# bobg/bs

Hardware: AMD Instinct MI355X
Metric: GiB/s device-resident split+ref-hash; chunk/ref bit-parity vs Go ref (higher is better)
Workload: dtype u8

## Files before the change

bs_amd/bsgpu.py:

```python
from __future__ import annotations

import contextlib
import ctypes
import os
import re

import numpy as np

_HERE = os.path.dirname(os.path.abspath(__file__))
LIB_PATH = os.environ.get("BSG_LIB_PATH") or os.path.join(_HERE, "libbsgpu.so")
HEADER_PATH = os.path.join(os.path.dirname(_HERE), "include", "bsgpu.h")

BSG_OK = 0
READ_SLACK = 256
ERRORS = {-22: "EINVAL", -12: "ENOMEM", -5: "EDEVICE", -71: "ESTATE", -19: "ENODEV",
          -2: "ENOTFOUND", -74: "ECORRUPT", -1001: "EIO"}


class BsgError(RuntimeError):
    def __init__(self, code: int, what: str = "", info: dict | None = None):
        self.code = code
        self.info = info
        super().__init__(f"{what}: bsgpu error {code} ({ERRORS.get(code, '?')})")

# ... 175 lines not shown
        return np.ascontiguousarray(ranges)
    out = np.zeros(len(ranges), dtype=READ_RANGE_DTYPE)
    for q, (root, offset, n) in enumerate(ranges):
        out[q]["root"] = np.frombuffer(bytes(root), dtype=np.uint8)
        out[q]["offset"], out[q]["len"] = offset, n
    return out

_lib = None


def exported_symbols_from_header(path: str = HEADER_PATH) -> list[str]:
    text = open(path).read()
    text = re.sub(r"/\*.*?\*/", "", text, flags=re.S)
    return sorted(set(re.findall(r"\b(bsg_[a-z0-9_]+)\s*\(", text)))


def lib() -> ctypes.CDLL:
    global _lib
    if _lib is not None:
        return _lib
    if not os.path.exists(LIB_PATH):
        raise RuntimeError(f"{LIB_PATH} not built: run `python -m bs_amd.build` "
                           "(the HIP path is the only path; there is no CPU fallback)")
    L = ctypes.CDLL(LIB_PATH)
    vp, u8p, u32p, u64p = (ctypes.c_void_p, ctypes.POINTER(ctypes.c_uint8),
                           ctypes.POINTER(ctypes.c_uint32), ctypes.POINTER(ctypes.c_uint64))
    sig = {
        "bsg_errstr": (ctypes.c_char_p, [ctypes.c_int]),
        "bsg_params_default": (Params, []),
        "bsg_default_table": (None, [u32p]),
        "bsg_device_count": (ctypes.c_int, []),
        "bsg_init": (ctypes.c_int, [ctypes.c_int]),
        "bsg_open": (vp, [ctypes.c_int, ctypes.POINTER(Params), u32p, ctypes.POINTER(ctypes.c_int)]),
        "bsg_write": (ctypes.c_int, [vp, vp, ctypes.c_size_t]),
        "bsg_close": (ctypes.c_int, [vp]),
        "bsg_close_begin": (ctypes.c_int, [vp]),
        "bsg_close_step": (ctypes.c_int, [vp, ctypes.POINTER(ctypes.c_size_t)]),
        "bsg_pending": (ctypes.c_size_t, [vp]),
        "bsg_drain": (ctypes.c_size_t, [vp, vp, ctypes.c_size_t]),
        "bsg_set_tile": (ctypes.c_int, [vp, ctypes.c_size_t]),
        "bsg_set_carry_cap": (ctypes.c_int, [vp, ctypes.c_size_t]),
        "bsg_write_window": (ctypes.c_int, [vp, ctypes.POINTER(ctypes.c_void_p),
                                            ctypes.POINTER(ctypes.c_size_t)]),
        "bsg_write_commit": (ctypes.c_int, [vp, ctypes.c_size_t]),
        "bsg_host_register": (ctypes.c_int, [vp, ctypes.c_size_t]),
        "bsg_host_unregister": (ctypes.c_int, [vp]),
        "bsg_write_pinned": (ctypes.c_int, [vp, vp, ctypes.c_size_t]),
        "bsg_free": (None, [vp]),
        "bsg_reset": (ctypes.c_int, [vp]),
        "bsg_engine_create": (vp, [ctypes.c_int, u32p, ctypes.POINTER(ctypes.c_int)]),
        "bsg_engine_destroy": (None, [vp]),
        "bsg_engine_run": (ctypes.c_int, [vp, vp, u64p, u64p, ctypes.c_uint32,
                                          ctypes.POINTER(Params)]),
        "bsg_engine_hash": (ctypes.c_int, [vp, vp, u64p, u64p, ctypes.c_uint32]),
        "bsg_engine_finish": (ctypes.c_int, [vp, u64p]),
        "bsg_engine_chunks_device": (vp, [vp]),
        "bsg_engine_copy_chunks": (ctypes.c_int, [vp, vp, ctypes.c_uint64]),
        "bsg_engine_copy_counts": (ctypes.c_int, [vp, u64p, ctypes.c_uint32]),
        "bsg_engine_stream": (vp, [vp]),
        "bsg_engine_trees": (ctypes.c_int, [vp, u64p, u64p]),
        "bsg_engine_copy_roots": (ctypes.c_int, [vp, vp, u64p, ctypes.c_uint32]),
        "bsg_engine_copy_tree_nodes": (ctypes.c_int, [vp, vp, ctypes.c_uint64, vp,
                                                      ctypes.c_uint64]),
        "bsg_engine_tree_nodes_device": (vp, [vp]),
        "bsg_engine_tree_arena_device": (vp, [vp]),
        "bsg_engine_roots_device": (vp, [vp]),
        "bsg_engine_trees_ms_debug": (ctypes.c_int, [vp, ctypes.POINTER(ctypes.c_float)]),
        "bsg_refset_new": (vp, [ctypes.c_int, ctypes.POINTER(ctypes.c_int)]),
        "bsg_refset_free": (None, [vp]),
        "bsg_refset_count": (ctypes.c_uint64, [vp]),
        "bsg_refset_add": (ctypes.c_int, [vp, vp, ctypes.c_uint64, vp]),
        "bsg_engine_dedup": (ctypes.c_int, [vp, vp, u64p, u64p]),
        "bsg_engine_copy_dedup": (ctypes.c_int, [vp, vp, ctypes.c_uint64, vp, vp,
                                                 ctypes.c_uint64]),
        "bsg_engine_dedup_first_device": (vp, [vp]),
        "bsg_engine_dedup_uniq_device": (vp, [vp]),
        "bsg_engine_dedup_pack_off_device": (vp, [vp]),
        "bsg_engine_pack_unique": (ctypes.c_int, [vp, vp, ctypes.c_uint64]),
        "bsg_engine_dedup_ms_debug": (ctypes.c_int, [vp, ctypes.POINTER(ctypes.c_float)]),
        "bsg_engine_restore": (ctypes.c_int, [vp, vp, ctypes.c_uint64, vp, ctypes.c_uint64, vp,
                                              ctypes.c_uint64, vp, ctypes.c_uint64, u64p, u64p,
                                              ctypes.c_uint32, ctypes.c_int,
                                              ctypes.POINTER(RestoreInfo)]),
        "bsg_engine_restore_ms_debug": (ctypes.c_int, [vp, ctypes.POINTER(ctypes.c_float)]),
        "bsg_engine_walk": (ctypes.c_int, [vp, vp, ctypes.c_uint64, vp, ctypes.c_uint64, vp,
                                           ctypes.c_uint32, ctypes.c_int, vp,
                                           ctypes.POINTER(WalkInfo)]),
        "bsg_engine_copy_walk": (ctypes.c_int, [vp, vp, ctypes.c_uint64, vp, vp,
                                                ctypes.c_uint32]),
        "bsg_engine_walk_records_device": (vp, [vp]),
        "bsg_engine_restore_walk": (ctypes.c_int, [vp, vp, ctypes.c_uint64, vp, ctypes.c_uint64,
                                                   vp, ctypes.c_uint64, u64p, ctypes.c_uint32,
                                                   ctypes.c_int, ctypes.POINTER(RestoreInfo)]),
        "bsg_engine_walk_ms_debug": (ctypes.c_int, [vp, ctypes.POINTER(ctypes.c_float)]),
        "bsg_engine_gc_mark": (ctypes.c_int, [vp, vp, ctypes.c_uint64, vp, ctypes.c_uint64, vp,
                                              ctypes.c_uint64, ctypes.c_int, vp,
                                              ctypes.POINTER(GcInfo)]),
        "bsg_engine_copy_gc": (ctypes.c_int, [vp, vp, ctypes.c_uint64, vp, ctypes.c_uint64,
                                              ctypes.c_int]),
        "bsg_engine_gc_live_device": (vp, [vp]),
        "bsg_engine_gc_compact": (ctypes.c_int, [vp, vp, ctypes.c_uint64, vp, ctypes.c_uint64,
                                                 ctypes.c_int, u64p]),
        "bsg_engine_gc_ms_debug": (ctypes.c_int, [vp, ctypes.POINTER(ctypes.c_float)]),
        "bsg_pool_new": (vp, [ctypes.c_int, ctypes.c_uint64, ctypes.c_uint64,
                              ctypes.POINTER(ctypes.c_int)]),
        "bsg_pool_free": (None, [vp]),
        "bsg_pool_stat": (ctypes.c_int, [vp, ctypes.POINTER(PoolStats)]),
        "bsg_pool_bytes_device": (vp, [vp]),
        "bsg_pool_table_device": (vp, [vp]),
        "bsg_pool_copy_table": (ctypes.c_int, [vp, vp, ctypes.c_uint64, ctypes.c_uint64]),
        "bsg_engine_pool_put": (ctypes.c_int, [vp, vp, ctypes.c_int,
                                               ctypes.POINTER(POOL_PUT_INFO)]),
        "bsg_pool_copy_where": (ctypes.c_int, [vp, vp, ctypes.c_uint64]),
        "bsg_pool_where_device": (vp, [vp]),
        "bsg_pool_put_ms_debug": (ctypes.c_int, [vp, ctypes.POINTER(ctypes.c_float)]),
        "bsg_pool_collect": (ctypes.c_int, [vp, vp, vp, vp, ctypes.c_uint64, ctypes.c_int, vp,
                                            ctypes.POINTER(PoolCollectInfo)]),
        "bsg_pool_copy_remap": (ctypes.c_int, [vp, vp, ctypes.c_uint64]),
        "bsg_pool_remap_device": (vp, [vp]),
        "bsg_pool_reset": (ctypes.c_int, [vp]),
        "bsg_pool_walk": (ctypes.c_int, [vp, vp, vp, ctypes.c_uint32, ctypes.c_int, vp,
                                         ctypes.POINTER(WalkInfo)]),
        "bsg_pool_restore_walk": (ctypes.c_int, [vp, vp, vp, ctypes.c_uint64, u64p,
                                                 ctypes.c_uint32, ctypes.c_int,
                                                 ctypes.POINTER(RestoreInfo)]),
        "bsg_engine_read": (ctypes.c_int, [vp, vp, ctypes.c_uint64, vp, ctypes.c_uint64, vp,
                                           ctypes.c_uint32, vp, ctypes.c_uint64, vp, ctypes.c_int,
                                           vp, vp, ctypes.POINTER(ReadInfo)]),
        "bsg_pool_read": (ctypes.c_int, [vp, vp, vp, ctypes.c_uint32, vp, ctypes.c_uint64, vp,
                                         ctypes.c_int, vp, vp, ctypes.POINTER(ReadInfo)]),
        "bsg_pool_kill_debug": (ctypes.c_int, [vp]),
        "bsg_engine_read_ms_debug": (ctypes.c_int, [vp, ctypes.POINTER(ctypes.c_float)]),
        "bsg_pool_collect_ms_debug": (ctypes.c_int, [vp, ctypes.POINTER(ctypes.c_float)]),
        "bsg_pool_merge": (ctypes.c_int, [vp, vp, vp, vp, ctypes.c_uint64, ctypes.c_int, vp,
                                          ctypes.POINTER(PoolMergeInfo)]),
        "bsg_pool_sync": (ctypes.c_int, [vp, vp, vp, ctypes.c_int, ctypes.POINTER(PoolMergeInfo)]),
        "bsg_pool_merge_ms_debug": (ctypes.c_int, [vp, ctypes.c_int,
                                                   ctypes.POINTER(ctypes.c_float)]),
        "bsg_pool_put_blobs": (ctypes.c_int, [vp, vp, vp, u64p, u64p, ctypes.c_uint64,
                                              ctypes.c_int, vp, ctypes.POINTER(POOL_PUT_INFO)]),
        "bsg_pool_get": (ctypes.c_int, [vp, vp, vp, ctypes.c_uint64, vp, ctypes.c_uint64,
                                        ctypes.c_int, vp, vp, ctypes.POINTER(PoolGetInfo)]),
        "bsg_pool_blobs_ms_debug": (ctypes.c_int, [vp, ctypes.POINTER(ctypes.c_float)]),
        "bsg_engine_pack_mode_debug": (ctypes.c_int, [vp, ctypes.c_int]),
        "bsg_engine_d2d_ms_debug": (ctypes.c_int, [vp, vp, vp, ctypes.c_uint64,
                                                   ctypes.POINTER(ctypes.c_float)]),
        "bsg_engine_candidates": (ctypes.c_uint64, [vp]),
        "bsg_engine_profile": (ctypes.c_int, [vp, ctypes.c_int]),
        "bsg_engine_diag": (ctypes.c_int, [vp, u64p]),
        "bsg_engine_timeline": (ctypes.c_int, [vp, u64p]),
        "bsg_engine_tiers_debug": (ctypes.c_int, [vp, u64p]),
        "bsg_engine_early_min_debug": (ctypes.c_int, [vp, ctypes.c_uint64]),
        "bsg_engine_host_tail": (ctypes.c_int, [vp, u64p]),
        "bsg_engine_host_tail_debug": (ctypes.c_int, [vp, ctypes.c_uint64, ctypes.c_uint32,
                                                      ctypes.c_int, ctypes.c_uint64]),
        "bsg_host_sha256_debug": (ctypes.c_int, [vp, ctypes.c_uint64, ctypes.c_int, vp]),
        "bsg_engine_early_picks_debug": (ctypes.c_int, [vp, u64p]),
        "bsg_engine_rescan_debug": (ctypes.c_uint64, [vp]),
        "bsg_engine_regions_debug": (ctypes.c_int, [vp, vp, ctypes.c_uint64]),
        "bsg_engine_stage_ms": (ctypes.c_int, [vp, ctypes.POINTER(ctypes.c_float)]),
        "bsg_split_hash_batch": (ctypes.c_int, [ctypes.c_int, vp, u64p, u64p, ctypes.c_uint32,
                                                ctypes.POINTER(Params), u32p, vp,
                                                ctypes.c_uint64, u64p, u64p]),
        "bsg_sha256_batch": (ctypes.c_int, [ctypes.c_int, vp, u64p, u64p, ctypes.c_uint32, vp]),
        "bsg_hasher_new": (vp, [ctypes.c_int]),
        "bsg_hasher_sum": (ctypes.c_int, [vp, vp, u64p, u64p, ctypes.c_uint32, vp]),
        "bsg_hasher_sum_ptrs": (ctypes.c_int, [vp, ctypes.POINTER(ctypes.c_void_p), u64p,
                                               ctypes.c_uint32, vp]),
        "bsg_hasher_free": (None, [vp]),
        "bsg_hasher_pinned_bytes": (ctypes.c_size_t, [vp]),
        "bsg_fill_splitmix": (ctypes.c_int, [ctypes.c_int, vp, ctypes.c_uint64, ctypes.c_uint64,
                                             vp]),
        "bsg_device_malloc": (vp, [ctypes.c_int, ctypes.c_size_t]),
        "bsg_device_free": (ctypes.c_int, [ctypes.c_int, vp]),
        "bsg_memcpy": (ctypes.c_int, [ctypes.c_int, vp, vp, ctypes.c_size_t, ctypes.c_int]),
        "bsg_device_synchronize": (ctypes.c_int, [ctypes.c_int]),
        "bsg_memstore_new": (vp, [ctypes.c_int]),
        "bsg_filestore_new": (vp, [ctypes.c_char_p, ctypes.c_int]),
        "bsg_store_free": (None, [vp]),
        "bsg_store_count": (ctypes.c_size_t, [vp]),
        "bsg_filestore_set_write_behind": (ctypes.c_int, [vp, ctypes.c_uint64]),
        "bsg_store_held_bytes": (ctypes.c_size_t, [vp]),
        "bsg_store_get": (ctypes.c_int, [vp, vp, vp, ctypes.c_size_t,
                                         ctypes.POINTER(ctypes.c_size_t)]),
        "bsg_store_put": (ctypes.c_int, [vp, vp, ctypes.c_size_t, vp,
                                         ctypes.POINTER(ctypes.c_int)]),
        "bsg_store_list": (ctypes.c_size_t, [vp, vp, ctypes.c_size_t]),
        "bsg_store_put_ref": (ctypes.c_int, [vp, vp, vp, ctypes.c_size_t,
                                             ctypes.POINTER(ctypes.c_int)]),
        "bsg_store_list_from": (ctypes.c_size_t, [vp, vp, vp, ctypes.c_size_t]),
        "bsg_store_delete": (ctypes.c_int, [vp, vp]),
        "bsg_split_protect": (ctypes.c_int, [vp, vp, vp, vp, ctypes.c_size_t,
                                             ctypes.POINTER(ctypes.c_size_t)]),
        "bsg_writer_new": (vp, [ctypes.c_int, vp, ctypes.POINTER(Params), ctypes.c_size_t,
                                ctypes.POINTER(ctypes.c_int)]),
        "bsg_writer_write": (ctypes.c_int, [vp, vp, ctypes.c_size_t]),
        "bsg_writer_close": (ctypes.c_int, [vp]),
        "bsg_writer_root": (ctypes.c_int, [vp, vp]),
        "bsg_writer_timings": (ctypes.c_int, [vp, ctypes.POINTER(ctypes.c_double)]),
        "bsg_stream_stats_get": (ctypes.c_int, [vp, ctypes.POINTER(StreamStats)]),
        "bsg_writer_free": (None, [vp]),
        "bsg_reader_new": (vp, [vp, vp, ctypes.POINTER(ctypes.c_int)]),
        "bsg_reader_open": (vp, [vp, vp, ctypes.c_int, ctypes.c_int, ctypes.POINTER(ctypes.c_int)]),
        "bsg_reader_read": (ctypes.c_int64, [vp, vp, ctypes.c_size_t]),
        "bsg_reader_seek": (ctypes.c_int64, [vp, ctypes.c_int64, ctypes.c_int]),
        "bsg_reader_size": (ctypes.c_uint64, [vp]),
        "bsg_reader_stats": (ctypes.c_int, [vp, u64p]),
        "bsg_debug_set": (ctypes.c_int, [ctypes.c_int, ctypes.c_int64]),
        "bsg_debug_get": (ctypes.c_int64, [ctypes.c_int]),
        "bsg_set_stream_base": (ctypes.c_int, [vp, ctypes.c_uint64]),
        "bsg_writer_set_stream_base": (ctypes.c_int, [vp, ctypes.c_uint64]),
        "bsg_reader_free": (None, [vp]),
    }
    partial = os.environ.get("BSG_LIB_PARTIAL") == "1"
    for name, (res, args) in sig.items():
        if partial and not hasattr(L, name):
            continue
        f = getattr(L, name)
        f.restype = res
        f.argtypes = args
    _lib = L
    return L


def _check(rc: int, what: str) -> None:
    if rc != BSG_OK:
        raise BsgError(rc, what)


def _as_u8(data) -> np.ndarray:
    if isinstance(data, np.ndarray):
        return np.ascontiguousarray(data.reshape(-1).view(np.uint8))
    return np.frombuffer(data, dtype=np.uint8)


def _u64(a) -> np.ndarray:
    return np.ascontiguousarray(np.asarray(a, dtype=np.uint64))


def _p(a: np.ndarray, ct):
    return a.ctypes.data_as(ctypes.POINTER(ct))


(KNOB_SEQ_WAIT, KNOB_LONG_MODE, KNOB_VERIFY_WINDOW, KNOB_EARLY, KNOB_POLL, KNOB_COPY_NT,
 KNOB_LIGHT_BYTES, KNOB_HOST_TAIL) = range(1, 9)


def debug_get(knob: int) -> int:
    return int(lib().bsg_debug_get(knob))


def debug_set(knob: int, value: int) -> None:
    _check(lib().bsg_debug_set(knob, value), "bsg_debug_set")


@contextlib.contextmanager
def debug_knob(knob: int, value: int):
    old = debug_get(knob)
    debug_set(knob, value)
    try:
        yield
    finally:
        debug_set(knob, old)


def device_count() -> int:
    return lib().bsg_device_count()


def init(device: int = 0) -> None:
    _check(lib().bsg_init(device), "bsg_init")


def default_table() -> np.ndarray:
    t = np.zeros(256, dtype=np.uint32)
    lib().bsg_default_table(_p(t, ctypes.c_uint32))
    return t


def params(bits: int = 16, min_size: int = 1024, fanout: int = 8) -> Params:
    return Params(bits, min_size, fanout, 0)


def _table_arg(table):
    if table is None:
        return None, None
    t = np.ascontiguousarray(np.asarray(table, dtype=np.uint32))
    assert t.shape == (256,)
    return t, _p(t, ctypes.c_uint32)


def split_hash_batch(streams: list[bytes] | list[np.ndarray], bits: int = 16,
                     min_size: int = 1024, table=None, device: int = 0):
    arrs = [np.frombuffer(bytes(s), dtype=np.uint8) if not isinstance(s, np.ndarray)
            else np.ascontiguousarray(s, dtype=np.uint8) for s in streams]
    lens = _u64([len(a) for a in arrs])
    off = _u64(np.concatenate([[0], np.cumsum(lens)[:-1]]) if len(arrs) else [])
    base = np.concatenate(arrs) if arrs else np.zeros(1, np.uint8)
    if base.size == 0:
        base = np.zeros(1, np.uint8)
    cap = int(sum(int(l) // (min_size or 64) + 2 for l in lens)) + 1
    out = np.zeros(cap, dtype=CHUNK_DTYPE)
    counts = np.zeros(max(len(arrs), 1), dtype=np.uint64)
    n = ctypes.c_uint64(0)
    p = params(bits, min_size)
    _t, tp = _table_arg(table)
# ... 349 lines not shown
                   cap: int | None = None):
        pp = pool.ptr if isinstance(pool, DeviceBuffer) else pool
        op = out.ptr if isinstance(out, DeviceBuffer) else out
        pool_bytes = pool.nbytes + READ_SLACK if pool_bytes is None else pool_bytes
        cap = out.nbytes if cap is None else cap
        n = ctypes.c_uint64(0)
        rc = lib().bsg_engine_gc_compact(self.h, pp, pool_bytes, op, cap,
                                         GC_ALIGN16 if align16 else 0, ctypes.byref(n))
        return rc, n.value

    def gc_ms(self) -> dict:
        out = (ctypes.c_float * 4)()
        _check(lib().bsg_engine_gc_ms_debug(self.h, out), "bsg_engine_gc_ms_debug")
        return {"index": float(out[0]), "levels": float(out[1]), "offsets": float(out[2]),
                "compact": float(out[3])}

    def pool_put(self, pool: "Pool", chunks: bool = True, nodes: bool = True) -> dict:
        flags = (POOL_CHUNKS if chunks else 0) | (POOL_NODES if nodes else 0)
        info = POOL_PUT_INFO()
        rc = lib().bsg_engine_pool_put(self.h, pool.h, flags, ctypes.byref(info))
        if rc != BSG_OK:
            raise BsgError(rc, "bsg_engine_pool_put", info.as_dict())
        pool._items = int(info.items)
        return info.as_dict()

    def pool_collect(self, src: "Pool", dst: "Pool", roots, flags: int = 0):
        roots = np.ascontiguousarray(np.frombuffer(roots, dtype=np.uint8)
                                     if isinstance(roots, (bytes, bytearray)) else roots,
                                     dtype=np.uint8).reshape(-1)
        assert len(roots) % 32 == 0
        nr = len(roots) // 32
        status = np.zeros(max(nr, 1), dtype=np.int32)
        info = PoolCollectInfo()
        nsrc = src.stat()["nblobs"] if src is not None and src.h else 0
        rc = lib().bsg_pool_collect(self.h, src.h if src is not None else None,
                                    dst.h if dst is not None else None, roots.ctypes.data, nr,
                                    flags, status.ctypes.data, ctypes.byref(info))
        self._gc_nblobs, self._gc_nlive = nsrc, int(info.gc.nlive)
        if rc == BSG_OK:
            dst._nremap = nsrc
        return rc, info.as_dict(), status[:nr]

    def pool_merge(self, src: "Pool", dst: "Pool", roots=None, all: bool = False,
                   verify: bool = False, missing_leaves: bool = False):
        if roots is None:
            rp, nr = None, 0
        else:
            roots = np.ascontiguousarray(np.frombuffer(roots, dtype=np.uint8)
                                         if isinstance(roots, (bytes, bytearray)) else roots,
                                         dtype=np.uint8).reshape(-1)
            assert len(roots) % 32 == 0
            rp, nr = roots.ctypes.data, len(roots) // 32
        flags = ((MERGE_ALL if all else 0) | (MERGE_VERIFY if verify else 0)
                 | (GC_MISSING_LEAVES if missing_leaves else 0))
        status = np.zeros(max(nr, 1), dtype=np.int32)
        info = PoolMergeInfo()
        nsrc = src.stat()["nblobs"] if src is not None and src.h else 0
        rc = lib().bsg_pool_merge(self.h, src.h if src is not None else None,
                                  dst.h if dst is not None else None, rp, nr, flags,
                                  status.ctypes.data, ctypes.byref(info))
        if not all:
            self._gc_nblobs, self._gc_nlive = nsrc, int(info.gc.nlive)
        if rc == BSG_OK:
            dst._nremap = nsrc
        return rc, info.as_dict(), status[:nr]

    def pool_sync(self, a: "Pool", b: "Pool", verify: bool = False):
        info = (PoolMergeInfo * 2)()
        na = a.stat()["nblobs"] if a is not None and a.h else 0
        nb = b.stat()["nblobs"] if b is not None and b.h else 0
        rc = lib().bsg_pool_sync(self.h, a.h if a is not None else None,
                                 b.h if b is not None else None, MERGE_VERIFY if verify else 0,
                                 info)
        if rc == BSG_OK:
            b._nremap, a._nremap = na, nb
        return rc, [info[0].as_dict(), info[1].as_dict()], np.zeros(0, dtype=np.int32)

    def pool_merge_ms(self, direction: int = 0) -> dict:
        out = (ctypes.c_float * 5)()
        _check(lib().bsg_pool_merge_ms_debug(self.h, direction, out), "bsg_pool_merge_ms_debug")
        return dict(zip(("probe", "plan", "verify", "append", "gather"), map(float, out)))

    def pool_walk(self, pool: "Pool", roots, flags: int = 0):
        roots = np.ascontiguousarray(np.frombuffer(roots, dtype=np.uint8)
                                     if isinstance(roots, (bytes, bytearray)) else roots,
                                     dtype=np.uint8).reshape(-1)
        assert len(roots) % 32 == 0
        ns = len(roots) // 32
        status = np.zeros(max(ns, 1), dtype=np.int32)
        info = WalkInfo()
        rc = lib().bsg_pool_walk(self.h, pool.h if pool is not None else None, roots.ctypes.data,
                                 ns, flags, status.ctypes.data, ctypes.byref(info))
        self._walk_ns, self._walk_nrecs = ns, int(info.nrecs)
        return rc, info.as_dict(), status[:ns]

    def pool_restore_walk(self, pool: "Pool", out, out_off, verify: bool = False,
                          out_cap: int | None = None):
        op = out.ptr if isinstance(out, DeviceBuffer) else out
        out_cap = out.nbytes if out_cap is None else out_cap
        oo = _u64(out_off)
        info = RestoreInfo()
        rc = lib().bsg_pool_restore_walk(self.h, pool.h if pool is not None else None, op, out_cap,
                                         _p(oo, ctypes.c_uint64), len(oo),
                                         RESTORE_VERIFY if verify else 0, ctypes.byref(info))
        return rc, info.as_dict()

    def read(self, pool, blobs, ranges, out, out_off, flags: int = 0,
             pool_bytes: int | None = None, out_cap: int | None = None):
        pp = pool.ptr if isinstance(pool, DeviceBuffer) else pool
        op = out.ptr if isinstance(out, DeviceBuffer) else out
        pool_bytes = pool.nbytes + READ_SLACK if pool_bytes is None else pool_bytes
        out_cap = out.nbytes if out_cap is None else out_cap
        blobs = np.ascontiguousarray(blobs, dtype=POOL_BLOB_DTYPE)
        rg, oo = read_ranges(ranges), _u64(out_off)
        assert len(rg) == len(oo)
        status = np.zeros(max(len(rg), 1), dtype=np.int32)
        got = np.zeros(max(len(rg), 1), dtype=np.uint64)
        info = ReadInfo()
        rc = lib().bsg_engine_read(self.h, pp, pool_bytes, blobs.ctypes.data, len(blobs),
                                   rg.ctypes.data, len(rg), op, out_cap, oo.ctypes.data, flags,
                                   status.ctypes.data, got.ctypes.data, ctypes.byref(info))
        return rc, status[:len(rg)], got[:len(rg)], info.as_dict()

    def read_ms(self) -> dict:
        out = (ctypes.c_float * 6)()
        _check(lib().bsg_engine_read_ms_debug(self.h, out), "bsg_engine_read_ms_debug")
        return dict(zip(("index", "levels", "placement", "resolve", "verify", "scatter"),
                        (float(x) for x in out)))

    def dedup_ms(self) -> dict:
        out = (ctypes.c_float * 2)()
        _check(lib().bsg_engine_dedup_ms_debug(self.h, out), "bsg_engine_dedup_ms_debug")
        return {"dedup": float(out[0]), "pack": float(out[1])}

    @property
    def stream(self) -> int:
        return lib().bsg_engine_stream(self.h) or 0

    def profile(self, enable: int = 1) -> None:
        _check(lib().bsg_engine_profile(self.h, int(enable)), "bsg_engine_profile")

    def stage_ms(self) -> list[float]:
        out = (ctypes.c_float * 3)()
        _check(lib().bsg_engine_stage_ms(self.h, out), "bsg_engine_stage_ms")
        return [float(x) for x in out]

    def diag(self) -> dict:
        d = np.zeros(16, dtype=np.uint64)
        _check(lib().bsg_engine_diag(self.h, _p(d, ctypes.c_uint64)), "bsg_engine_diag")
        out = {"nlong": int(d[0]), "long_thresh": int(d[1]), "max_nblocks": int(d[2]),
               "nshort": int(d[13]), "wave_tickets": int(d[14]), "total_blocks": int(d[15])}
        t = np.zeros(4, dtype=np.uint64)
        _check(lib().bsg_engine_timeline(self.h, _p(t, ctypes.c_uint64)), "bsg_engine_timeline")
        if t[0] and t[1] and t[3]:
            t0 = int(t[0])
            out["timeline_us"] = {"long_start": round((int(t[1]) - t0) * 0.01, 1),
                                  "long_end": round((int(t[2]) - t0) * 0.01, 1),
                                  "lane_end": round((int(t[3]) - t0) * 0.01, 1)}
        if os.environ.get("BSG_DIAG_RAW") == "1":
            out["diag2_raw"] = [int(x) for x in d[8:13]]
        for tag, o in (("long", 3), ("lane", 8)):
            cyc, rt, nb = int(d[o + 1] - d[o]), int(d[o + 3] - d[o + 2]), int(d[o + 4])
            if nb and rt:
                out[tag] = {"blocks": nb, "cycles_per_block": round(cyc / nb, 1),
                            "clock_ghz": round(cyc / (rt * 10.0), 3),
                            "us_per_block": round(rt * 0.01 / nb, 4)}
        t = np.zeros(12, dtype=np.uint64)
        _check(lib().bsg_engine_host_tail(self.h, _p(t, ctypes.c_uint64)), "bsg_engine_host_tail")
        out["host_tail"] = {"chunks": int(t[0]), "bytes": int(t[1]), "cut_blocks": int(t[2]),
                            "gather_us": int(t[3]), "host_done_us": int(t[4]),
                            "impl": "x86-sha" if int(t[5]) == 1 else "portable",
                            "threads": int(t[6]), "host_rate_bytes_s": int(t[7]),
                            "longest_blocks": int(t[8]), "longest_left_blocks": int(t[9]),
                            "host_blocks": int(t[10]), "cpuid_sha": bool(t[11])}
        return out

    def set_host_tail(self, min_bytes: int = 512 << 20, force_cut: int = 0,
                      portable: bool = False, ring_bytes: int = 0) -> None:
        _check(lib().bsg_engine_host_tail_debug(self.h, int(min_bytes), int(force_cut),
                                                int(bool(portable)), int(ring_bytes)),
               "bsg_engine_host_tail_debug")

    def tiers(self) -> dict:
        d = np.zeros(6, dtype=np.uint64)
        _check(lib().bsg_engine_tiers_debug(self.h, _p(d, ctypes.c_uint64)),
               "bsg_engine_tiers_debug")
        return {"nlong_grp": int(d[0]), "tickets_grp": int(d[1]), "helped": int(d[2]),
                "wave_tickets": int(d[3]), "early": (bool(d[4]), bool(d[5]))}

    def set_early_min(self, nbytes: int) -> None:
        _check(lib().bsg_engine_early_min_debug(self.h, int(nbytes)),
               "bsg_engine_early_min_debug")

    def early_picks(self) -> list:
        d = np.zeros(4, dtype=np.uint64)
        _check(lib().bsg_engine_early_picks_debug(self.h, _p(d, ctypes.c_uint64)),
               "bsg_engine_early_picks_debug")
        out = []
        for k in range(2):
            top, idx = int(d[k]), int(d[2 + k])
            if top:
                out.append((top >> 32, top & 0xFFFFFFFF, idx - 1 if idx else None))
            elif idx:
                raise BsgError(-5, f"bsg_engine_early_picks_debug: idx[{k}] without top[{k}]")
        if not d[0] and d[1]:
            raise BsgError(-5, "bsg_engine_early_picks_debug: top[1] without top[0]")
        return out

    def regions(self) -> dict:
        kmax = 256
        d = np.zeros(8 + kmax + kmax + 1, dtype=np.uint64)
        _check(lib().bsg_engine_regions_debug(self.h, d.ctypes.data, d.nbytes),
               "bsg_engine_regions_debug")
        R = int(d[0])
        if not 1 <= R <= kmax:
            raise BsgError(-5, f"bsg_engine_regions_debug: nregions {R}")
        return {"nregions": R, "off": [int(x) for x in d[8 + kmax: 8 + kmax + R + 1]]}

    @property
    def candidates(self) -> int:
        return lib().bsg_engine_candidates(self.h)

    @property
    def rescan_strips(self) -> int:
        return int(lib().bsg_engine_rescan_debug(self.h))

    def close(self) -> None:
        if self.h:
            lib().bsg_engine_destroy(self.h)
            self.h = None

    def __del__(self):
        try:
            self.close()
        except Exception:
            pass


IN_SET = 1 << 63


class RefSet:

    def __init__(self, device: int = 0):
        err = ctypes.c_int(0)
        self.h = lib().bsg_refset_new(device, ctypes.byref(err))
        if not self.h:
            raise BsgError(err.value, "bsg_refset_new")

    def add(self, refs) -> np.ndarray:
        if not isinstance(refs, np.ndarray):
            refs = np.frombuffer(b"".join(bytes(r) for r in refs), dtype=np.uint8)
        a = np.ascontiguousarray(refs, dtype=np.uint8).reshape(-1, 32)
        added = np.zeros(max(len(a), 1), dtype=np.uint8)
        _check(lib().bsg_refset_add(self.h, a.ctypes.data, len(a), added.ctypes.data),
               "bsg_refset_add")
        return added[: len(a)]

    def count(self) -> int:
        return int(lib().bsg_refset_count(self.h))

    def free(self) -> None:
        if self.h:
            lib().bsg_refset_free(self.h)
            self.h = None

    def __del__(self):
        try:
            self.free()
        except Exception:
            pass


class Pool:

    def __init__(self, cap_bytes: int, cap_blobs: int, device: int = 0):
        err = ctypes.c_int(0)
        self.device, self._items, self._nremap = device, 0, 0
        self.h = lib().bsg_pool_new(device, cap_bytes, cap_blobs, ctypes.byref(err))
        if not self.h:
            raise BsgError(err.value, "bsg_pool_new")

    def stat(self) -> dict:
        st = PoolStats()
        _check(lib().bsg_pool_stat(self.h, ctypes.byref(st)), "bsg_pool_stat")
        return st.as_dict()

    @property
    def ptr(self) -> int:
        return lib().bsg_pool_bytes_device(self.h) or 0

    @property
    def pool_bytes(self) -> int:
        return self.stat()["pool_bytes"]

    def table(self, first: int = 0) -> np.ndarray:
        n = self.stat()["nblobs"] - first
        out = np.zeros(max(n, 1), dtype=POOL_BLOB_DTYPE)
        _check(lib().bsg_pool_copy_table(self.h, out.ctypes.data, first, max(n, 0)),
               "bsg_pool_copy_table")
        return out[:max(n, 0)]

    def where(self) -> np.ndarray:
        out = np.zeros(max(self._items, 1), dtype=np.uint64)
        _check(lib().bsg_pool_copy_where(self.h, out.ctypes.data, self._items),
               "bsg_pool_copy_where")
        return out[:self._items]

    def to_host(self, n: int | None = None) -> np.ndarray:
        n = self.stat()["bytes"] if n is None else n
        out = np.empty(max(n, 1), dtype=np.uint8)
        if n:
            _check(lib().bsg_memcpy(self.device, out.ctypes.data, self.ptr, n, 1), "bsg_memcpy")
        return out[:n]

    def read(self, eng: "Engine", ranges, out, out_off, flags: int = 0,
             out_cap: int | None = None):
        op = out.ptr if isinstance(out, DeviceBuffer) else out
        out_cap = out.nbytes if out_cap is None else out_cap
        rg, oo = read_ranges(ranges), _u64(out_off)
        assert len(rg) == len(oo)
        status = np.zeros(max(len(rg), 1), dtype=np.int32)
        got = np.zeros(max(len(rg), 1), dtype=np.uint64)
        info = ReadInfo()
        rc = lib().bsg_pool_read(eng.h if eng is not None else None, self.h, rg.ctypes.data,
                                 len(rg), op, out_cap, oo.ctypes.data, flags, status.ctypes.data,
                                 got.ctypes.data, ctypes.byref(info))
        return rc, status[:len(rg)], got[:len(rg)], info.as_dict()
# ... 372 lines not shown
```

bs_amd/csrc/bsgpu_host.cpp:

```cpp
#include <hip/hip_runtime.h>
#include <pthread.h>
#include <sched.h>
#include <sys/mman.h>
#include <sys/syscall.h>
#include <unistd.h>

#include <emmintrin.h>

#include <algorithm>
#include <atomic>
#include <chrono>
#include <condition_variable>
#include <cstdio>
#include <cstdlib>
#include <cstring>
#include <deque>
#include <functional>
#include <memory>
#include <mutex>
#include <new>
#include <thread>
#include <vector>

#include "../../include/bsgpu.h"
// ... 868 lines not shown
  HCHECK(hipEventCreate(&a));
  if (hipEventCreate(&b) != hipSuccess) {
    (void)hipGetLastError();
    (void)hipEventDestroy(a);
    return BSG_EDEVICE;
  }
  hipError_t err = hipEventRecord(a, e->stream);
  if (err == hipSuccess)
    err = hipMemcpyDtoDAsync((hipDeviceptr_t)dst, (hipDeviceptr_t)src, n, e->stream);
  if (err == hipSuccess) err = hipEventRecord(b, e->stream);
  if (err == hipSuccess) err = hipStreamSynchronize(e->stream);
  if (err == hipSuccess) err = hipEventElapsedTime(ms, a, b);
  (void)hipEventDestroy(a);
  (void)hipEventDestroy(b);
  if (err != hipSuccess) (void)hipGetLastError();
  return herr(err);
}

bsg_refset* bsg_refset_new(int device, int* err) {
  int dummy;
  if (!err) err = &dummy;
  if (device < 0 || device >= bsg_device_count()) {
    *err = BSG_ENODEV;
    return nullptr;
  }
  bsg_refset* s = new (std::nothrow) bsg_refset();
  if (!s) {
    *err = BSG_ENOMEM;
    return nullptr;
  }
  s->dev = device;
  *err = BSG_EDEVICE;
  if (hipSetDevice(device) == hipSuccess && stream_acquire(device, &s->stream) == hipSuccess) {
    s->num_cus = device_cus(device);
    s->slots = kRefSetSlots0;
    s->key_cap = kRefSetSlots0;
    *err = BSG_ENOMEM;
    if (s->tab.ensure(8 * s->slots) == hipSuccess && s->keys.ensure(32 * s->key_cap) == hipSuccess) {
      *err = herr(hipMemset(s->tab.p, 0xFF, 8 * s->slots));
      if (*err == BSG_OK) return s;
    }
  }
  (void)hipGetLastError();
  bsg_refset_free(s);
  return nullptr;
}

void bsg_refset_free(bsg_refset* s) {
  if (!s) return;
  hipSetDevice(s->dev);
  if (s->stream) {
    hipStreamSynchronize(s->stream);
    stream_release(s->dev, s->stream);
  }
  delete s;
}

uint64_t bsg_refset_count(const bsg_refset* s) { return s ? s->count.load() : 0; }

int bsg_refset_add(bsg_refset* s, const uint8_t* refs, uint64_t n, uint8_t* added) {
  if (!s || (n && !refs) || n > (1ull << 40)) return BSG_EINVAL;
  std::lock_guard<std::mutex> g(s->mu);
  if (s->dead) return BSG_ESTATE;
  HCHECK(hipSetDevice(s->dev));
  if (!n) return BSG_OK;
  int rc;
  if ((rc = s->work.reserve(n))) return rc;
  MCHECK(s->staged.ensure(32 * n));
  HCHECK(hipMemcpyAsync(s->staged.p, refs, 32 * n, hipMemcpyHostToDevice, s->stream));
  HCHECK(hipMemsetAsync(s->work.hdr.p, 0, sizeof(DedupHdr), s->stream));
  HCHECK(s->work.tab.clear(s->stream));
  DedupArgs a = s->work.args(s->staged.as<uint8_t>(), 32, nullptr, 0, n);
  s->lookup_args(&a);
  HCHECK(dbg("launch_dedup", s->stream, launch_dedup(a, s->stream, s->num_cus)));
  if ((rc = s->work.readback(s->stream))) {
    if (rc == BSG_EDEVICE) s->dead = true;
    return rc;
  }
  const uint64_t m = s->work.last.nunique;
  if (m > n) {
    s->dead = true;
    return BSG_EDEVICE;
  }
  std::vector<uint64_t> first;
  if (added) {
    try {
      first.resize(n);
    } catch (const std::bad_alloc&) {
      return BSG_ENOMEM;
    }
    HCHECK(hipMemcpy(first.data(), s->work.first.p, 8 * n, hipMemcpyDeviceToHost));
  }
  if ((rc = s->add_new(a, m, &s->work, s->stream))) return rc;
  if (added)
    for (uint64_t i = 0; i < n; ++i) added[i] = first[i] == i ? 1 : 0;
  return BSG_OK;
}

int bsg_engine_profile(bsg_engine* e, int enable) {
  if (!e || enable < 0 || enable > 2) return BSG_EINVAL;
  int rc = e->setdev();
  if (rc) return rc;
  if (enable) HCHECK(e->marks.create(4));
  e->profile = enable;
  return BSG_OK;
}

int bsg_engine_stage_ms(const bsg_engine* e, float out[3]) {
  if (!e || !out || !e->profile) return BSG_EINVAL;
  for (int i = 0; i < 3; ++i) out[i] = e->stage_ms[i];
  return BSG_OK;
}

uint64_t bsg_engine_candidates(const bsg_engine* e) { return e ? e->last.ncand : 0; }

int bsg_engine_diag(const bsg_engine* e, uint64_t out[16]) {
  if (!e || !out) return BSG_EINVAL;
  out[0] = e->last.nlong;
  out[1] = e->last.long_thresh;
  out[2] = e->last.max_nblocks;
  for (int i = 0; i < 5; ++i) out[3 + i] = e->last.diag[i];
  for (int i = 0; i < 5; ++i) out[8 + i] = e->last.diag2[i];
  out[13] = e->last.nshort;
  out[14] = e->last.ntickets;
  out[15] = e->last.total_blocks;
  return BSG_OK;
}

int bsg_engine_host_tail(const bsg_engine* e, uint64_t out[12]) {
  if (!e || !out) return BSG_EINVAL;
  const bsg_engine::TailStat& t = e->tail_stat;
  out[0] = t.chunks;
  out[1] = t.bytes;
  out[2] = t.cut;
  out[3] = (uint64_t)(t.gather_ms > 0 ? t.gather_ms * 1000.f : 0.f);
  out[4] = (uint64_t)std::max<int64_t>(0, t.host_done_us);
  out[5] = (uint64_t)t.impl;
  out[6] = (uint64_t)t.threads;
  out[7] = (uint64_t)t.host_rate;
  out[8] = t.longest_all;
  out[9] = t.longest_left;
  out[10] = t.blocks;
  out[11] = sha256_have_x86() ? 1 : 0;
  return BSG_OK;
}

extern "C" int bsg_engine_host_tail_debug(bsg_engine* e, uint64_t min_bytes, uint32_t force_cut,
                                          int portable, uint64_t ring_bytes) {
  if (!e || e->enqueued || (ring_bytes && ring_bytes < 4096)) return BSG_EINVAL;
  e->tail_min = min_bytes;
  e->tail_force_cut = force_cut;
  e->tail_portable = portable != 0;
  e->tail_ring_force = ring_bytes;
  return BSG_OK;
}

extern "C" int bsg_engine_regions_debug(bsg_engine* e, void* out, uint64_t nbytes) {
  if (!e || !out || !e->regions.p) return BSG_EINVAL;
  if (e->setdev()) return BSG_EDEVICE;
  const uint64_t n = std::min<uint64_t>(nbytes, sizeof(Regions));
  if (hipStreamSynchronize(e->stream) != hipSuccess) return BSG_EDEVICE;
  return hipMemcpy(out, e->regions.p, n, hipMemcpyDeviceToHost) == hipSuccess ? BSG_OK : BSG_EDEVICE;
}

static int read_early(bsg_engine* e, Early* ea) {
  if (e->hash_mode || !e->ctr.p || e->ctr.cap < sizeof(Counters) + sizeof(Early)) return BSG_OK;
  if (e->setdev() || hipStreamSynchronize(e->stream) != hipSuccess ||
      hipMemcpy(ea, e->dearly(), sizeof(Early), hipMemcpyDeviceToHost) != hipSuccess)
    return BSG_EDEVICE;
  return BSG_OK;
}

extern "C" int bsg_engine_tiers_debug(bsg_engine* e, uint64_t out[6]) {
  if (!e || !out || e->enqueued) return BSG_EINVAL;
  out[0] = e->last.nlong_grp;
  out[1] = e->last.tickets_grp;
  out[2] = e->last.helped;
  out[3] = e->last.ntickets;
  Early ea{};
  const int rc = read_early(e, &ea);
  for (int k = 0; k < kEarly; ++k) out[4 + k] = (ea.top[k] && ea.idx[k]) ? 1 : 0;
  return rc;
}

extern "C" int bsg_engine_early_min_debug(bsg_engine* e, uint64_t bytes) {
  if (!e || e->enqueued) return BSG_EINVAL;
  e->early_min = bytes;
  return BSG_OK;
}

extern "C" int bsg_engine_early_picks_debug(bsg_engine* e, uint64_t out[4]) {
  if (!e || !out || e->enqueued) return BSG_EINVAL;
  Early ea{};
  const int rc = read_early(e, &ea);
  for (int k = 0; k < kEarly; ++k) {
    out[k] = ea.top[k];
    out[kEarly + k] = ea.idx[k];
  }
  return rc;
}

extern "C" uint64_t bsg_engine_rescan_debug(const bsg_engine* e) {
  return e && !e->enqueued ? e->last.rescan : ~0ull;
}

extern "C" int bsg_engine_trees_ms_debug(const bsg_engine* e, float out[4]) {
  if (!e || !out) return BSG_EINVAL;
  if (!e->profile || !e->tree.valid) return BSG_ESTATE;
  for (int i = 0; i < 4; ++i) out[i] = e->tree.ms[i];
  return BSG_OK;
}

int bsg_engine_timeline(const bsg_engine* e, uint64_t out[4]) {
  if (!e || !out) return BSG_EINVAL;
  out[0] = e->last.sha_start_rt;
  out[1] = e->last.diag[2];
  out[2] = e->last.diag[3];
  out[3] = e->last.lane_end_rt;
  return BSG_OK;
}

bsg_ctx* bsg_open(int device, const bsg_params* params, const uint32_t* table, int* err) {
  int dummy;
  if (!err) err = &dummy;
  Params p;
  bsg_params norm;
  int rc = normalize(params, &p, &norm);
  if (rc) {
    *err = rc;
    return nullptr;
  }
  if (device < 0 || device >= bsg_device_count()) {
    *err = BSG_ENODEV;
    return nullptr;
  }
  bsg_ctx* c = new (std::nothrow) bsg_ctx();
  if (!c) {
    *err = BSG_ENOMEM;
    return nullptr;
  }
  c->params = norm;
  c->p = p;
  if (hipSetDevice(device) != hipSuccess || (rc = c->init(device, table)) != BSG_OK) {
    delete c;
    *err = rc ? rc : BSG_EDEVICE;
    return nullptr;
  }
  *err = BSG_OK;
  return c;
}

int bsg_set_tile(bsg_ctx* c, size_t tile) {
  if (!c || tile < 4096 || c->fill || c->pos != c->stream0 || c->started) return BSG_EINVAL;
  c->tile = tile;
  return BSG_OK;
}

int bsg_set_carry_cap(bsg_ctx* c, size_t bytes) {
  if (!c || c->fill || c->pos != c->stream0 || c->started || bytes > 0xffffffffull)
    return BSG_EINVAL;
  c->carry_cap = bytes;
  return BSG_OK;
}

int bsg_set_stream_base(bsg_ctx* c, uint64_t base) {
  if (!c || c->fill || c->pos != c->stream0 || c->started || c->closed) return BSG_EINVAL;
  c->stream0 = c->pos = base;
  return BSG_OK;
}

static int ctx_write(bsg_ctx* c, const uint8_t* p, size_t n,
                     int (bsg_ctx::*write)(const uint8_t*, size_t)) {
  if (!c) return BSG_EINVAL;
  if (c->closed) return BSG_ESTATE;
  if (c->sticky) return c->sticky;
  if (n && !p) return BSG_EINVAL;
  if (hipSetDevice(c->dev) != hipSuccess) return BSG_EDEVICE;
  c->started = true;
  int rc = (c->*write)(p, n);
  if (rc) c->sticky = rc;
  return rc;
}

int bsg_write(bsg_ctx* c, const uint8_t* p, size_t n) { return ctx_write(c, p, n, &bsg_ctx::write); }

int bsg_host_register(void* p, size_t n) {
  if (!p || !n) return BSG_EINVAL;
  HCHECK(hipHostRegister(p, n, hipHostRegisterDefault));
  return BSG_OK;
}

int bsg_host_unregister(void* p) {
  if (!p) return BSG_EINVAL;
  HCHECK(hipHostUnregister(p));
  return BSG_OK;
}

int bsg_write_pinned(bsg_ctx* c, const uint8_t* p, size_t n) {
  return ctx_write(c, p, n, &bsg_ctx::write_pinned);
}

int bsg_write_window(bsg_ctx* c, uint8_t** p, size_t* cap) {
  if (!c || !p || !cap) return BSG_EINVAL;
  if (c->closed) return BSG_ESTATE;
  if (c->sticky) return c->sticky;
  if (hipSetDevice(c->dev) != hipSuccess) return BSG_EDEVICE;
// ... 316 lines not shown
```

bs_amd/csrc/bsgpu_internal.h:

```cpp
#pragma once
#include <stddef.h>
#include <stdint.h>

namespace bsg {

constexpr int kScanWG = 512;
#ifndef BSG_STRIP
#define BSG_STRIP 2048
#endif
constexpr int kStrip = BSG_STRIP;
constexpr int kSlotCap = 4;
constexpr int kTabRows = 256;
constexpr int kTabRep = 64;

constexpr int kCandPosShift = 8;
constexpr uint64_t kCandPosMask = (1ull << 40) - 1;
constexpr uint64_t kCandForce = 1ull << 7;

__host__ __device__ inline uint64_t cand_pack(uint32_t stream, uint64_t pos, bool force,
                                              uint32_t tz) {
  return ((uint64_t)stream << 48) | ((pos & kCandPosMask) << kCandPosShift) |
         (force ? kCandForce : 0ull) | (uint64_t)(tz & 63u);
}
__host__ __device__ inline uint32_t cand_stream(uint64_t c) { return (uint32_t)(c >> 48); }
__host__ __device__ inline uint64_t cand_pos(uint64_t c) {
  return (c >> kCandPosShift) & kCandPosMask;
}
__host__ __device__ inline bool cand_force(uint64_t c) { return (c & kCandForce) != 0; }
__host__ __device__ inline uint32_t cand_tz(uint64_t c) { return (uint32_t)(c & 63u); }

__host__ __device__ inline uint32_t slot_pack(uint32_t local, bool force, uint32_t tz) {
  return (local << 8) | (force ? 0x80u : 0u) | (tz & 63u);
}

struct StreamDesc {
  uint64_t data_off;
  uint64_t len;
  uint64_t strip0;
  uint64_t seg_base;
  uint64_t open_start;
  uint64_t consumed;
  uint32_t finalize;
  uint32_t prefix_len;
  uint32_t mid[8];
  uint32_t carry_cap;
  uint32_t flags;
  uint8_t hist[64];
};
constexpr uint32_t kDescOpenInDevice = 1;
static_assert(sizeof(StreamDesc) == 160, "StreamDesc layout");

struct CarryOut {
  uint32_t mid[8];
  uint64_t consumed;
  uint64_t open_start;
  uint32_t prefix_len;
  uint32_t valid;
};

struct ChunkRec {
  uint64_t offset;
  uint64_t len;
  uint32_t level;
  uint32_t stream;
  uint8_t ref[32];
};
static_assert(sizeof(ChunkRec) == 56, "ChunkRec layout");

struct Params {
  uint32_t split_bits;
  uint32_t min_size;
  uint32_t mask;
  uint32_t pad_;
};

struct Counters {
  uint64_t ncand;
  uint64_t nchunks;
  uint64_t help_wg;
  uint64_t overflow;
  uint64_t error;
  uint64_t max_nblocks;
  uint64_t long_thresh;
  uint64_t nlong;
  uint64_t long_head;
  uint64_t nshort;
  uint64_t bucket_width;
  uint64_t diag[5];
  uint64_t diag2[5];
  uint64_t rescan;
  uint64_t total_blocks;
  uint64_t long_buckets;
  uint64_t ntickets;
  uint64_t sha_arrivals;
  uint64_t sha_start_rt;
  uint64_t lane_end_rt;
  uint64_t nlong_grp;
  uint64_t tickets_grp;
  uint64_t nrefine;
  uint64_t helped;
  uint64_t scan_ticket;
  uint64_t pad[7];
};
static_assert(sizeof(Counters) == 320, "Counters layout");

struct LaneJob {
  uint64_t dptr;
  uint64_t start;
  uint64_t len;
  uint32_t stream;
  uint32_t meta;
};
static_assert(sizeof(LaneJob) == 32, "LaneJob layout");
constexpr uint32_t kLaneJobSlow = 0x80000000u;

constexpr uint32_t kMaxRegions = 256;
constexpr uint32_t kRegionSegs = 256;
constexpr uint32_t kMinRegionJobs = 4096;
constexpr uint64_t kRegionBytes = 1ull << 30;
struct Regions {
  uint64_t nregions;
  uint64_t rr;
  uint64_t pad_[6];
  uint64_t head[kMaxRegions];
  uint64_t off[kMaxRegions + 1];
  uint64_t pad2_[7];
  uint32_t cnt[kRegionSegs * kMaxRegions];
};

constexpr int kEarly = 2;
struct Early {
  uint64_t top[kEarly];
  uint64_t idx[kEarly];
  uint64_t diag[5];
  uint64_t pad_;
  ChunkRec rec[kEarly];
};
static_assert(sizeof(Early) % 16 == 0, "Early layout");

constexpr uint32_t kTailBuckets = 256;
constexpr uint32_t kTailMaxItems = 4096;
constexpr uint32_t kTailMinBlocks = 256;
constexpr uint32_t kTailSlotAlign = 256;
struct TailItem {
  uint64_t job;
  uint64_t start;
  uint64_t len;
  uint64_t off;
  uint32_t stream;
  uint32_t level;
};
static_assert(sizeof(TailItem) == 40, "TailItem layout");
struct TailHdr {
  uint64_t count;
  uint64_t cutb;
  uint64_t bytes;
  uint64_t blocks;
  uint64_t mx_all;
  uint64_t mx_left;
  uint64_t ring_head;
  uint64_t taken;
  uint32_t cnt[kTailBuckets];
  uint32_t maxb[kTailBuckets];
  uint64_t rbytes[kTailBuckets];
  uint64_t nblk[kTailBuckets];
  uint32_t base[kTailBuckets];
  uint32_t fill[kTailBuckets];
};
static_assert(sizeof(TailHdr) % 16 == 0, "TailHdr layout");
constexpr uint32_t kTailMetaWords = 8;
__host__ __device__ inline uint64_t tail_slot(uint64_t len) {
  return (len + 16 + kTailSlotAlign - 1) & ~(uint64_t)(kTailSlotAlign - 1);
}

constexpr uint32_t kLongMinBlocks = 1024;
#ifndef BSG_SOLO
#define BSG_SOLO 16
#endif
constexpr uint32_t kSolo = BSG_SOLO;
constexpr uint32_t kGroup = 8;
constexpr uint32_t kPairGroup = 32;
constexpr int kLongRow = 68;
constexpr int kRingWords = 65 * kLongRow;
constexpr int kLptBuckets = 4096;
constexpr uint64_t kReadSlack = 256;

constexpr uint32_t kTreeMaxHeights = 40;
struct TreeNode {
  uint64_t blob_off;
  uint32_t blob_len;
  uint32_t stream;
  uint32_t height;
  uint32_t reserved;
  uint8_t ref[32];
};
static_assert(sizeof(TreeNode) == 56, "TreeNode layout");
struct TreeHdr {
  uint64_t nnodes;
  uint64_t arena_bytes;
  uint64_t max_r;
  uint64_t error;
  uint64_t hoff[kTreeMaxHeights + 1];
};
struct TreeNodeMeta {
  uint64_t child0;
  uint64_t nchild;
  uint64_t offset, size;
  uint64_t out_idx;
  uint64_t blob_off;
  uint32_t blob_len;
  uint32_t stream;
};

constexpr uint64_t kDedupEmpty = ~0ull;
constexpr uint64_t kDedupInSet = 1ull << 63;
constexpr uint64_t kRefSetSlots0 = 1024;
constexpr uint64_t kRefSetLoadPct = 50;
constexpr uint32_t kPackTile = 32768;
struct DedupHdr {
  uint64_t error;
  uint64_t nunique;
  uint64_t unique_bytes;
  uint64_t pad_;
};

constexpr uint32_t kRestoreTile = 32768;
struct PoolBlob {
  uint64_t off;
  uint64_t len;
  uint8_t ref[32];
};
static_assert(sizeof(PoolBlob) == 48, "PoolBlob layout");
struct RestoreHdr {
  DedupHdr dd;
  uint64_t invalid;
  uint64_t missing;
  uint64_t mismatch;
  uint64_t bad_blob;
};
static_assert(sizeof(RestoreHdr) == 64, "RestoreHdr layout");

constexpr uint32_t kWalkMaxDepth = 64;
constexpr uint32_t kWalkRuns = 12;
constexpr uint64_t kWalkDead = ~0ull;
constexpr uint32_t kWalkCorrupt = 1;
constexpr uint32_t kWalkNotFound = 2;
struct WalkItem {
  uint64_t blob;
  uint64_t exp_off;
  uint64_t exp_size;
  uint64_t parent;
  uint32_t stream;
  uint32_t flags;
};
constexpr uint32_t kWalkNoCover = 1;
static_assert(sizeof(WalkItem) == 40, "WalkItem layout");
struct WalkNode {
  uint64_t nchild;
  uint64_t offset, size;
  uint64_t nrec;
  uint64_t rbase;
  uint32_t kind;
  uint32_t nruns;
  uint64_t run_pos[kWalkRuns];
  uint64_t run_idx[kWalkRuns];
  uint32_t run_len[kWalkRuns];
};
struct WalkHdr {
  DedupHdr dd;
  uint64_t nnodes;
  uint64_t depth;
  uint64_t lvl_all[kWalkMaxDepth + 1];
  uint64_t lvl_nodes[kWalkMaxDepth + 1];
};
static_assert(sizeof(WalkHdr) % 16 == 0, "WalkHdr layout");

struct ReadHdr {
  WalkHdr w;
  RestoreHdr r;
  uint64_t verified;
  uint64_t pad_;
};
static_assert(sizeof(ReadHdr) % 16 == 0 && offsetof(ReadHdr, r) % 16 == 0, "ReadHdr layout");

constexpr uint32_t kGcClaimed = 1;
constexpr uint32_t kGcFailed = 2;
constexpr uint32_t kGcTile = 32768;
struct GcHdr {
  WalkHdr w;
  uint64_t bad_form;
  uint64_t bad_miss;
  uint64_t verdict;
  uint64_t leaf_miss;
  uint64_t missing_leaves;
  uint64_t end, end16;
  uint64_t size0;
  uint32_t status0;
  uint32_t pad_;
  uint64_t pad2_;
  uint8_t zero[16];
};
static_assert(sizeof(GcHdr) % 16 == 0 && offsetof(GcHdr, zero) % 16 == 0, "GcHdr layout");

constexpr uint32_t kPoolTile = 32768;
struct PoolHdr {
  DedupHdr dd;
  uint64_t total16;
  uint64_t last_len;
  uint64_t known;
  uint64_t repeats;
  uint8_t zero[16];
};
static_assert(sizeof(PoolHdr) % 16 == 0 && offsetof(PoolHdr, zero) % 16 == 0, "PoolHdr layout");

struct MergeHdr {
  GcHdr g;
  RestoreHdr r;
  uint64_t selected;
  uint64_t known;
  uint64_t added_bytes;
  uint64_t end;
  uint64_t verified;
  uint64_t pad_;
// ... 19 lines not shown
```

bs_amd/csrc/bsgpu_kernels.hip:

```cpp
#include <hip/hip_runtime.h>

#include <algorithm>

#include "bsgpu_internal.h"
#include "bsgpu_launch.h"
#include "sha256_device.h"
#include "scan_block_loop.inc"

#ifndef BSG_TLEN_PCT
#define BSG_TLEN_PCT 55
#endif
#ifndef BSG_PAIR_PCT
#define BSG_PAIR_PCT 34
#endif
#ifndef BSG_TLEN_PCT_LIGHT
#define BSG_TLEN_PCT_LIGHT 48
#endif
#ifndef BSG_PAIR_PCT_LIGHT
#define BSG_PAIR_PCT_LIGHT 30
#endif

namespace bsg {

typedef uint32_t u32x4 __attribute__((ext_vector_type(4), aligned(4)));
// ... 1260 lines not shown

__global__ __launch_bounds__(kRegionSegs) void k_rscan(ShaArgs a) {
  __shared__ uint32_t wsum[kRegionSegs / 64];
  if (a.ctr->overflow || a.ctr->error || a.ctr->nchunks > a.chunk_cap) return;
  const uint32_t r = blockIdx.x, t = threadIdx.x;
  if (r >= a.reg->nregions) return;
  uint32_t* c = a.reg->cnt + t * kMaxRegions + r;
  const uint32_t v = *c;
  uint32_t x = v;
  for (int o = 1; o < 64; o <<= 1) {
    const uint32_t y = __shfl_up(x, o);
    if ((t & 63) >= (uint32_t)o) x += y;
  }
  if ((t & 63) == 63) wsum[t >> 6] = x;
  __syncthreads();
  uint32_t base = 0, tot = 0;
  for (uint32_t w = 0; w < kRegionSegs / 64; ++w) {
    if (w < (t >> 6)) base += wsum[w];
    tot += wsum[w];
  }
  *c = base + x - v;
  if (t == 0) a.reg->head[r] = tot;
}

__global__ __launch_bounds__(kMaxRegions) void k_rtotal(ShaArgs a) {
  __shared__ uint64_t wsum[kMaxRegions / 64];
  if (a.ctr->overflow || a.ctr->error || a.ctr->nchunks > a.chunk_cap) return;
  const uint32_t t = threadIdx.x;
  const uint32_t R = (uint32_t)a.reg->nregions;
  const uint64_t v = t < R ? a.reg->head[t] : 0;
  uint64_t x = v;
  for (int o = 1; o < 64; o <<= 1) {
    const uint64_t y = __shfl_up(x, o);
    if ((t & 63) >= (uint32_t)o) x += y;
  }
  if ((t & 63) == 63) wsum[t >> 6] = x;
  __syncthreads();
  uint64_t base = 0;
  for (uint32_t w = 0; w < (t >> 6); ++w) base += wsum[w];
  __syncthreads();
  a.reg->off[t] = t < R ? base + x - v : a.ctr->nshort;
  if (t == 0) {
    a.reg->off[kMaxRegions] = a.ctr->nshort;
    a.reg->rr = 0;
  }
  a.reg->head[t] = 0;
}

__global__ __launch_bounds__(256) void k_rscatter(ShaArgs a) {
  __shared__ uint64_t base[kMaxRegions];
  __shared__ uint32_t tc[kMaxRegions];
  if (a.ctr->overflow || a.ctr->error || a.ctr->nchunks > a.chunk_cap) return;
  const uint64_t n = a.ctr->nshort, L = seg_len(n);
  const uint32_t t = threadIdx.x;
  base[t] = a.reg->off[t] + a.reg->cnt[blockIdx.x * kMaxRegions + t];
  tc[t] = 0;
  __syncthreads();
  const uint64_t lo = blockIdx.x * L, hi = min(n, lo + L);
  for (uint64_t tile = lo; tile < hi; tile += 256) {
    const uint64_t i = tile + t;
    uint32_t r = 0, rank = 0;
    uint64_t j = 0;
    if (i < hi) {
      r = a.oreg[i];
      j = a.order[i];
      rank = atomicAdd(&tc[r], 1u);
    }
    __syncthreads();
    if (i < hi) a.rorder[base[r] + rank] = j;
    __syncthreads();
    base[t] += tc[t];
    tc[t] = 0;
    __syncthreads();
  }
}

__global__ __launch_bounds__(1024) void k_bucket_scan(ShaArgs a) {
  __shared__ uint32_t wsum[16];
  __shared__ uint32_t nok;
  const uint32_t t = threadIdx.x;
  if (t == 0) nok = 0;
  const uint64_t mx = a.ctr->max_nblocks, w = a.ctr->bucket_width;
  const bool light = a.ctr->total_blocks * 10ull < mx * 64ull * a.waves;
  uint64_t tlen = (mx * (light ? BSG_TLEN_PCT_LIGHT : BSG_TLEN_PCT)) / 100;
  const uint64_t share = (a.ctr->total_blocks * 9) / (10ull * 64ull * a.waves);
  tlen = max(max(tlen, share), (uint64_t)kLongMinBlocks);
  uint64_t cap = kSolo + (uint64_t)kGroup * (a.waves / 2 > kSolo ? a.waves / 2 - kSolo : 0);
  if (a.long_mode == 2) { tlen = 0; cap = ~0ull; }
  uint32_t e[4], pe[4];
#pragma unroll
  for (int i = 0; i < 4; ++i) e[i] = a.bucket_elig[4 * t + i];
  block_scan4(e, pe, wsum);
  uint32_t ok = 0;
#pragma unroll
  for (int i = 0; i < 4; ++i) {
    const uint64_t b = 4 * t + i;
    const uint64_t top = mx > b * w ? mx - b * w : 0;
    ok += (a.long_mode != 1 && top >= tlen && (uint64_t)pe[i] + e[i] <= cap) ? 1u : 0u;
  }
  __syncthreads();
  atomicAdd(&nok, ok);
  __syncthreads();
  const uint32_t nlb8 = nok;
  uint32_t lv[4], lo[4], sv[4], so[4];
#pragma unroll
  for (int i = 0; i < 4; ++i) lv[i] = (4 * t + i < nlb8) ? e[i] : 0u;
  const uint32_t n8 = block_scan4(lv, lo, wsum);
  const uint64_t t8 = n8 <= kSolo ? n8 : kSolo + (n8 - kSolo + kGroup - 1) / kGroup;
  uint32_t nlb = nlb8;
  const uint64_t pair_pct = light ? BSG_PAIR_PCT_LIGHT : BSG_PAIR_PCT;
  if (pair_pct > 0 && a.long_mode == 0) {
    const uint64_t tlen2 = max((mx * pair_pct) / 100, (uint64_t)kLongMinBlocks);
    const uint64_t tb = a.waves / 2 > t8 ? a.waves / 2 - t8 : 0;
    const uint64_t cap2 = tb * kPairGroup;
    uint32_t ok2 = 0;
#pragma unroll
    for (int i = 0; i < 4; ++i) {
      const uint64_t b = 4 * t + i;
      const uint64_t top = mx > b * w ? mx - b * w : 0;
      ok2 += (b >= nlb8 && top >= tlen2 && (uint64_t)pe[i] + e[i] - n8 <= cap2) ? 1u : 0u;
    }
    __syncthreads();
    if (t == 0) nok = 0;
    __syncthreads();
    atomicAdd(&nok, ok2);
    __syncthreads();
    nlb = nlb8 + nok;
#pragma unroll
    for (int i = 0; i < 4; ++i) lv[i] = (4 * t + i < nlb) ? e[i] : 0u;
  }
  const uint32_t nlong = block_scan4(lv, lo, wsum);
#pragma unroll
  for (int i = 0; i < 4; ++i) sv[i] = a.bucket_cnt[4 * t + i] - lv[i];
  const uint32_t nshort = block_scan4(sv, so, wsum);
#pragma unroll
  for (int i = 0; i < 4; ++i) {
    a.bucket_loff[4 * t + i] = lo[i];
    a.bucket_off[4 * t + i] = so[i];
  }
  if (t == 0) {
    a.ctr->long_buckets = nlb;
    a.ctr->nlong = nlong;
    a.ctr->nshort = nshort;
    const uint64_t rmax = min((uint64_t)kMaxRegions, max((uint64_t)a.waves / 16, (uint64_t)1));
    const uint64_t rspan = (a.span + kRegionBytes - 1) / kRegionBytes;
    a.reg->nregions = min(min(rmax, rspan), max((uint64_t)nshort / kMinRegionJobs, (uint64_t)1));
    if (a.span <= kRegionBytes) {
      a.reg->off[0] = 0;
      a.reg->off[1] = nshort;
      a.reg->head[0] = 0;
    }
    a.ctr->long_thresh = mx > (uint64_t)nlb * w ? mx - (uint64_t)nlb * w : 0;
    a.ctr->nlong_grp = n8;
    a.ctr->tickets_grp = t8;
    const uint64_t helped = (light && a.long_mode == 0)
                                ? min(min((uint64_t)n8, (uint64_t)kSolo), (uint64_t)a.waves / 2)
                                : 0;
    a.ctr->helped = helped;
    a.ctr->long_head = helped;
    a.ctr->ntickets = t8 + (nlong - n8 + kPairGroup - 1) / kPairGroup;
  }
}

__device__ __forceinline__ bool early_key(const ShaArgs& a, int k, uint32_t* s, uint64_t* start,
                                          uint64_t* end) {
  const uint64_t top = a.early->top[k];
  if (!top) return false;
  const uint64_t c = a.cand[(uint32_t)top], cn = a.cand[(uint32_t)top + 1];
  *s = cand_stream(c);
  const uint64_t sb = a.streams[*s].seg_base;
  *start = sb + cand_pos(c) + 1;
  *end = sb + cand_pos(cn) + 1;
  return true;
}

__global__ __launch_bounds__(256) void k_lens(ShaArgs a) {
  if (a.ctr->overflow || a.ctr->error) return;
  const uint64_t M = a.ctr->nchunks;
  if (M > a.chunk_cap) return;
  const uint64_t njobs = M + a.nstreams;
  const uint64_t stride = (uint64_t)gridDim.x * blockDim.x;
  uint32_t st[8];
  ShaJob jb;
  uint64_t mx = 0, tot = 0;
  uint32_t es[kEarly] = {~0u, ~0u};
  uint64_t e0[kEarly] = {0, 0}, e1[kEarly] = {0, 0};
  if (a.early)
    for (int k = 0; k < kEarly; ++k)
      if (!early_key(a, k, &es[k], &e0[k], &e1[k])) es[k] = ~0u;
  for (uint64_t j = (uint64_t)blockIdx.x * blockDim.x + threadIdx.x; j < njobs; j += stride) {
    uint32_t info = kNoJob;
    if (sha_setup(a, j, M, jb, st)) {
      tot += jb.nblocks;
      if (jb.prefix == 0) mx = max(mx, (uint64_t)jb.nblocks);
      bool early = false;
      if (j < M && jb.fin && jb.prefix == 0 && jb.consumed == 0)
        for (int k = 0; k < kEarly; ++k)
          if (jb.stream == es[k] && jb.start == e0[k] && jb.end == e1[k]) {
            a.early->idx[k] = j + 1;
            early = true;
          }
      if (early) {
        a.jinfo[j] = kNoJob;
        continue;
      }
      info = min(jb.nblocks, ~kJobElig) | (jb.prefix == 0 ? kJobElig : 0u);
      LaneJob d;
      d.dptr = reinterpret_cast<uint64_t>(jb.dbase);
      d.start = jb.start;
      d.len = jb.L;
      d.stream = jb.stream;
      d.meta = jb.level | ((jb.fin && jb.prefix == 0 && jb.consumed == 0) ? 0u : kLaneJobSlow);
      a.jdesc[j] = d;
    }
    a.jinfo[j] = info;
  }
  __shared__ uint64_t wmx[4], wtot[4];
  for (int o = 32; o > 0; o >>= 1) {
    mx = max(mx, (uint64_t)__shfl_down(mx, o));
    tot += (uint64_t)__shfl_down(tot, o);
  }
  if ((threadIdx.x & 63) == 0) {
    wmx[threadIdx.x >> 6] = mx;
    wtot[threadIdx.x >> 6] = tot;
  }
  __syncthreads();
  if (threadIdx.x == 0) {
    for (int w = 1; w < 4; ++w) {
      mx = max(mx, wmx[w]);
      tot += wtot[w];
    }
    if (mx) atomicMax(reinterpret_cast<unsigned long long*>(&a.ctr->max_nblocks), (unsigned long long)mx);
    if (tot) atomicAdd(reinterpret_cast<unsigned long long*>(&a.ctr->total_blocks), (unsigned long long)tot);
  }
}

__global__ void k_thresh(Counters* ctr, int mode) {
  (void)mode;
  const uint64_t w = (ctr->max_nblocks + kLptBuckets) / kLptBuckets;
  ctr->bucket_width = w ? w : 1;
}

__device__ __forceinline__ void ring_sync() {
  __builtin_amdgcn_fence(__ATOMIC_SEQ_CST, "wavefront");
  __builtin_amdgcn_wave_barrier();
}

__device__ __forceinline__ uint32_t wave_max(uint32_t v) {
  for (int o = 32; o > 0; o >>= 1) v = max(v, (uint32_t)__shfl_xor((int)v, o));
  return v;
}

__device__ void sha_wave_job(const ShaArgs& a, uint64_t M, uint64_t t, uint64_t nlong,
                             uint32_t* ring) {
  const uint32_t lane = threadIdx.x & 63u;
  const uint64_t n8 = a.ctr->nlong_grp, t8 = a.ctr->tickets_grp;
  const bool pairs = t >= t8;
  const bool solo = !pairs && t < kSolo;
  const uint64_t j0 = solo ? t : pairs ? n8 + (t - t8) * kPairGroup : kSolo + (t - kSolo) * kGroup;
  const uint64_t jend = pairs ? nlong : n8;
  const uint32_t G = solo ? 1u : pairs ? kPairGroup : kGroup;
  const uint32_t B = 64u / G;
  const uint32_t cA = lane / B;
  const uint32_t cR = cA;
  ShaJob ja;
  uint32_t sta[8];
  const bool va = j0 + cA < jend && sha_setup(a, a.long_list[j0 + cA], M, ja, sta);
  if (!va) {
    ja.dbase = a.data;
    ja.L = 0;
    ja.fin = 0;
    ja.consumed = 0;
  }
  const uint32_t na = va ? ja.nblocks : 0u;
  ShaJob jb;
  uint32_t st[8];
  const bool vb = j0 + cR < jend && sha_setup(a, a.long_list[j0 + cR], M, jb, st);
  const uint32_t nb = vb ? jb.nblocks : 0u;
  uint64_t tm0 = 0, tr0 = 0;
  const bool stamp = t == 0 && !(a.early && a.early->top[0]);
  if (stamp) {
    tm0 = __builtin_amdgcn_s_memtime();
    tr0 = __builtin_amdgcn_s_memrealtime();
  }
  const uint32_t nmax = __builtin_amdgcn_readfirstlane(wave_max(nb));
  const SkewLane bl = skew_lane();
  const OctLane ol = oct_lane();
  const bool a_side = pairs ? bl.a_side : ol.a_side;
  uint32_t hs[4];
  hs[0] = a_side ? st[0] : st[6];
  hs[1] = a_side ? st[1] : st[7];
  hs[2] = a_side ? st[2] : st[4];
  hs[3] = a_side ? st[3] : st[5];
  RawBlock rb;
  raw_load(ja.dbase, 64ull * min(lane % B, max(na, 1u) - 1u), 0, ja.L, rb);
  for (uint32_t base = 0; base < nmax; base += B) {
    const uint32_t blk = min(base + lane % B, max(na, 1u) - 1u);
    uint32_t W[16];
    raw_to_words(rb, W);
    const int32_t valid = rb.valid;
    raw_load(ja.dbase, 64ull * min(base + B + lane % B, max(na, 1u) - 1u), 0, ja.L, rb);
    if (valid < 64) {
      pad_words(valid, W);
      if (ja.fin && blk + 1 == na) {
        const uint64_t bits = (ja.consumed + ja.L) * 8ull;
        W[14] = (uint32_t)(bits >> 32);
        W[15] = (uint32_t)bits;
      }
    }
    u32x4a* row = reinterpret_cast<u32x4a*>(ring + lane * kLongRow);
#pragma unroll
    for (int tt = 0; tt < 64; tt += 4) {
      uint32_t kw[4];
#pragma unroll
      for (int u = 0; u < 4; ++u) {
        const int i = tt + u;
        if (i >= 16) {
          const uint32_t w15 = W[(i - 15) & 15], w2 = W[(i - 2) & 15];
          const uint32_t s0 = xor3(rotr(w15, 7), rotr(w15, 18), w15 >> 3);
          const uint32_t s1 = xor3(rotr(w2, 17), rotr(w2, 19), w2 >> 10);
          W[i & 15] = (W[i & 15] + s0) + (W[(i - 7) & 15] + s1);
        }
        kw[u] = kK256[i] + W[i & 15];
      }
      row[tt / 4] = u32x4a{kw[0], kw[1], kw[2], kw[3]};
    }
    ring_sync();
    const uint32_t steps = min(B, nmax - base);
    const uint32_t* ones = ring + 64 * kLongRow;
    const uint32_t* krow = a_side ? ones : ring + cR * B * kLongRow;
    const uint32_t stride = a_side ? 0u : 4u * kLongRow;
    if (pairs)
      sha256_blocks_skew(hs, krow, stride, steps, (int32_t)nb - (int32_t)base, bl);
    else
      sha256_blocks_oct(hs, krow, stride, steps, (int32_t)nb - (int32_t)base, ol);
    ring_sync();
  }
  const int pe = (int)(lane & ~(B - 1u)), pa = (int)((lane & ~(B - 1u)) | (pairs ? 1u : 4u));
#pragma unroll
  for (int k = 0; k < 4; ++k) st[k] = (uint32_t)__shfl((int)hs[k], pa);
  st[6] = (uint32_t)__shfl((int)hs[0], pe);
  st[7] = (uint32_t)__shfl((int)hs[1], pe);
  st[4] = (uint32_t)__shfl((int)hs[2], pe);
  st[5] = (uint32_t)__shfl((int)hs[3], pe);
  if (vb && (lane & (B - 1u)) == 0) {
    sha_finish(a, jb, st);
    if (stamp) {
      a.ctr->diag[1] = __builtin_amdgcn_s_memtime();
      a.ctr->diag[3] = __builtin_amdgcn_s_memrealtime();
      a.ctr->diag[0] = tm0;
      a.ctr->diag[2] = tr0;
      a.ctr->diag[4] = jb.nblocks;
    }
  }
}

__device__ __forceinline__ uint64_t pop_uniform(uint64_t* head) {
  uint32_t lo = 0, hi = 0;
  if ((threadIdx.x & 63u) == 0) {
    const uint64_t t = atomicAdd(reinterpret_cast<unsigned long long*>(head), 1ull);
    lo = (uint32_t)t;
    hi = (uint32_t)(t >> 32);
  }
  lo = __builtin_amdgcn_readlane(lo, 0);
  hi = __builtin_amdgcn_readlane(hi, 0);
  return ((uint64_t)hi << 32) | lo;
}

constexpr uint32_t kHelpHalfWords = 64 * kLongRow;
constexpr uint32_t kHelpOnes = 4 * kHelpHalfWords;
constexpr uint32_t kHelpFlags = kHelpOnes + kLongRow;
constexpr uint32_t kHelpWords = kHelpFlags + 8;
constexpr uint32_t kHelpSlot = 4 * kRingWords;

__device__ __forceinline__ uint32_t lds_seq_load(uint32_t* p) {
  return __hip_atomic_load(p, __ATOMIC_ACQUIRE, __HIP_MEMORY_SCOPE_WORKGROUP);
}
__device__ __forceinline__ void lds_seq_store(uint32_t* p, uint32_t v) {
  __hip_atomic_store(p, v, __ATOMIC_RELEASE, __HIP_MEMORY_SCOPE_WORKGROUP);
}
__device__ bool lds_seq_wait(const ShaArgs& a, uint32_t* p, uint32_t want) {
  for (uint32_t i = 0; i < a.seq_wait_limit; ++i) {
    if ((uint32_t)__builtin_amdgcn_readfirstlane((int)lds_seq_load(p)) == want) return true;
    __builtin_amdgcn_s_sleep(1);
  }
  if ((threadIdx.x & 63u) == 0)
    atomicOr(reinterpret_cast<unsigned long long*>(&a.ctr->error), 8ull);
  return false;
}

__device__ __forceinline__ bool solo_chain_blocks(const ShaArgs& a, uint32_t nb, uint32_t (&st)[8],
                                                  uint32_t* lds, uint32_t c) {
  const uint32_t lane = threadIdx.x & 63u;
  const OctLane ol = oct_lane();
  uint32_t hs[4];
  hs[0] = ol.a_side ? st[0] : st[6];
  hs[1] = ol.a_side ? st[1] : st[7];
  hs[2] = ol.a_side ? st[2] : st[4];
  hs[3] = ol.a_side ? st[3] : st[5];
  uint32_t* fill_seq = lds + kHelpFlags + 2 * c;
  uint32_t* done_seq = lds + kHelpFlags + 4 + 2 * c;
  const uint32_t* ones = lds + kHelpOnes;
  uint32_t f = 0;
  for (uint32_t base = 0; base < nb; base += 64, ++f) {
    const uint32_t h = f & 1u;
    if (!lds_seq_wait(a, fill_seq + h, f / 2 + 1)) return false;
    const uint32_t* krow = ol.a_side ? ones : lds + (2 * c + h) * kHelpHalfWords;
    const uint32_t stride = ol.a_side ? 0u : 4u * kLongRow;
    sha256_blocks_oct_solo(hs, krow, stride, min(64u, nb - base), ol);
    if (lane == 0) lds_seq_store(done_seq + h, f / 2 + 1);
  }
#pragma unroll
  for (int k = 0; k < 4; ++k) st[k] = (uint32_t)__shfl((int)hs[k], 4);
  st[6] = (uint32_t)__shfl((int)hs[0], 0);
  st[7] = (uint32_t)__shfl((int)hs[1], 0);
  st[4] = (uint32_t)__shfl((int)hs[2], 0);
  st[5] = (uint32_t)__shfl((int)hs[3], 0);
  return true;
}

__device__ void sha_solo_chain(const ShaArgs& a, uint64_t M, uint64_t t, uint32_t* lds,
                               uint32_t c) {
  const uint32_t lane = threadIdx.x & 63u;
  ShaJob jb;
  uint32_t st[8];
  const bool vb = sha_setup(a, a.long_list[t], M, jb, st);
  const uint32_t nb = __builtin_amdgcn_readfirstlane(vb ? jb.nblocks : 0u);
  const bool stamp = t == 0 && !(a.early && a.early->top[0]);
  uint64_t tm0 = 0, tr0 = 0;
  if (stamp) {
    tm0 = __builtin_amdgcn_s_memtime();
    tr0 = __builtin_amdgcn_s_memrealtime();
  }
  if (!solo_chain_blocks(a, nb, st, lds, c)) return;
  if (vb && lane == 0) {
    sha_finish(a, jb, st);
    if (stamp) {
      a.ctr->diag[1] = __builtin_amdgcn_s_memtime();
      a.ctr->diag[3] = __builtin_amdgcn_s_memrealtime();
      a.ctr->diag[0] = tm0;
      a.ctr->diag[2] = tr0;
      a.ctr->diag[4] = jb.nblocks;
    }
  }
}

__device__ __forceinline__ void solo_fill_blocks(const ShaArgs& a, ShaJob ja, bool va,
                                                 uint32_t* lds, uint32_t c) {
  const uint32_t lane = threadIdx.x & 63u;
  if (!va) {
    ja.dbase = a.data;
    ja.L = 0;
    ja.fin = 0;
    ja.consumed = 0;
  }
  const uint32_t na = __builtin_amdgcn_readfirstlane(va ? ja.nblocks : 0u);
  uint32_t* fill_seq = lds + kHelpFlags + 2 * c;
  uint32_t* done_seq = lds + kHelpFlags + 4 + 2 * c;
  RawBlock rb;
  raw_load(ja.dbase, 64ull * min(lane, max(na, 1u) - 1u), 0, ja.L, rb);
  uint32_t f = 0;
  for (uint32_t base = 0; base < na; base += 64, ++f) {
    const uint32_t h = f & 1u;
    if (f >= 2 && !lds_seq_wait(a, done_seq + h, f / 2)) return;
    const uint32_t blk = min(base + lane, max(na, 1u) - 1u);
    uint32_t W[16];
    raw_to_words(rb, W);
    const int32_t valid = rb.valid;
    raw_load(ja.dbase, 64ull * min(base + 64u + lane, max(na, 1u) - 1u), 0, ja.L, rb);
    if (valid < 64) {
      pad_words(valid, W);
      if (ja.fin && blk + 1 == na) {
        const uint64_t bits = (ja.consumed + ja.L) * 8ull;
        W[14] = (uint32_t)(bits >> 32);
        W[15] = (uint32_t)bits;
      }
    }
    u32x4a* row = reinterpret_cast<u32x4a*>(lds + (2 * c + h) * kHelpHalfWords + lane * kLongRow);
#pragma unroll
    for (int tt = 0; tt < 64; tt += 4) {
      uint32_t kw[4];
#pragma unroll
      for (int u = 0; u < 4; ++u) {
        const int i = tt + u;
        if (i >= 16) {
          const uint32_t w15 = W[(i - 15) & 15], w2 = W[(i - 2) & 15];
          const uint32_t s0 = xor3(rotr(w15, 7), rotr(w15, 18), w15 >> 3);
          const uint32_t s1 = xor3(rotr(w2, 17), rotr(w2, 19), w2 >> 10);
          W[i & 15] = (W[i & 15] + s0) + (W[(i - 7) & 15] + s1);
        }
        kw[u] = kK256[i] + W[i & 15];
      }
      row[tt / 4] = u32x4a{kw[0], kw[1], kw[2], kw[3]};
    }
    if (lane == 0) lds_seq_store(fill_seq + h, f / 2 + 1);
  }
}

__device__ void sha_solo_fill(const ShaArgs& a, uint64_t M, uint64_t t, uint32_t* lds,
                              uint32_t c) {
  ShaJob ja;
  uint32_t sta[8];
  const bool va = sha_setup(a, a.long_list[t], M, ja, sta);
  solo_fill_blocks(a, ja, va, lds, c);
}

constexpr uint32_t kShaWaves = 4;
constexpr uint32_t kShaBlock = 64 * kShaWaves;

template <bool HELP>
__global__ __launch_bounds__(kShaBlock, 1) void k_sha(ShaArgs a) {
  extern __shared__ __attribute__((aligned(16))) uint32_t lds[];
  if (a.ctr->overflow || a.ctr->error) return;
  if ((a.ctr->helped != 0) != HELP) return;
  const uint64_t M = a.ctr->nchunks;
  if (M > a.chunk_cap) return;
  const uint64_t nlong = a.ctr->nlong;
  if ((threadIdx.x & 63u) == 0) {
    const uint64_t rt = __builtin_amdgcn_s_memrealtime();
    if (atomicAdd(reinterpret_cast<unsigned long long*>(&a.ctr->sha_arrivals), 1ull) == 0)
      a.ctr->sha_start_rt = rt;
  }
  const uint64_t ntickets = a.ctr->ntickets;
  const uint32_t wv = __builtin_amdgcn_readfirstlane(threadIdx.x >> 6);
  uint32_t* ring = lds + wv * kRingWords;
  uint64_t t = ~0ull;
  bool helper_wg = false;
  if constexpr (HELP) {
    if (threadIdx.x == 0)
      lds[kHelpSlot] = (uint32_t)atomicAdd(reinterpret_cast<unsigned long long*>(&a.ctr->help_wg), 1ull);
    __syncthreads();
    const uint64_t helped = a.ctr->helped, hw = lds[kHelpSlot];
    if (hw * 2 < helped) {
      helper_wg = true;
      for (uint32_t i = threadIdx.x; i < (uint32_t)kLongRow; i += blockDim.x) lds[kHelpOnes + i] = 1u;
      if (threadIdx.x < 8) lds[kHelpFlags + threadIdx.x] = 0u;
      __syncthreads();
      const uint32_t c = wv & 1u;
      const uint64_t ht = hw * 2 + c;
      if (ht < helped) {
        __builtin_amdgcn_s_setprio(3);
        if (wv < 2) sha_solo_chain(a, M, ht, lds, c);
        else sha_solo_fill(a, M, ht, lds, c);
        __builtin_amdgcn_s_setprio(0);
      }
    }
  }
  if (!helper_wg) {
    for (uint32_t i = threadIdx.x & 63u; i < (uint32_t)kLongRow; i += 64) ring[64 * kLongRow + i] = 1u;
    t = pop_uniform(&a.ctr->long_head);
  }
  if (t < ntickets) {
    __builtin_amdgcn_s_setprio(3);
    while (t < ntickets) {
      sha_wave_job(a, M, t, nlong, ring);
      t = pop_uniform(&a.ctr->long_head);
    }
    __builtin_amdgcn_s_setprio(0);
  }
  sha_lane_mode(a, M);
  if ((threadIdx.x & 63u) == 0)
    atomicMax(reinterpret_cast<unsigned long long*>(&a.ctr->lane_end_rt),
              (unsigned long long)__builtin_amdgcn_s_memrealtime());
}

__device__ __forceinline__ uint64_t pick_key(const uint64_t* __restrict__ cand, uint64_t n,
                                             uint64_t i, uint64_t minsz) {
  if (i == 0 || i + 1 >= n) return 0;
  const uint64_t c = cand[i];
  const uint64_t cp = cand[i - 1], cn = cand[i + 1];
  const uint32_t s = cand_stream(c);
  if (cand_stream(cp) != s || cand_stream(cn) != s) return 0;
  const uint64_t E = cand_pos(c) + 1, Ep = cand_pos(cp) + 1, En = cand_pos(cn) + 1;
  if (E - Ep < minsz) return 0;
  if (!cand_force(cn) && En - E < minsz) return 0;
  if (cand_force(c)) return 0;
  const uint64_t nb = (En - E + 8) / 64 + 1;
  if (nb < kLongMinBlocks || nb >= (1ull << 31)) return 0;
  return (nb << 32) | i;
}

__device__ __forceinline__ void top2_wave(uint64_t& b1, uint64_t& b2) {
  uint64_t m1 = b1;
  for (int o = 32; o > 0; o >>= 1) m1 = max(m1, (uint64_t)__shfl_xor((long long)m1, o));
  uint64_t m2 = b1 == m1 ? b2 : b1;
  for (int o = 32; o > 0; o >>= 1) m2 = max(m2, (uint64_t)__shfl_xor((long long)m2, o));
  b1 = m1;
  b2 = m2;
}

constexpr uint32_t kPickWGs = 64;
__global__ __launch_bounds__(1024) void k_pick(const uint64_t* __restrict__ cand, Counters* ctr,
                                               uint32_t min_size, Early* e) {
  __shared__ uint64_t wp[2 * 16];
  if (ctr->overflow || ctr->error) return;
  const uint64_t n = ctr->ncand;
  if (n >= (1ull << 32)) return;
  uint64_t b1 = 0, b2 = 0;
  const uint64_t stride = (uint64_t)gridDim.x * blockDim.x;
  for (uint64_t i = (uint64_t)blockIdx.x * blockDim.x + threadIdx.x; i < n; i += stride) {
    const uint64_t key = pick_key(cand, n, i, min_size);
    b2 = max(b2, min(key, b1));
    b1 = max(b1, key);
  }
  top2_wave(b1, b2);
  const uint32_t w = threadIdx.x >> 6, nw = blockDim.x >> 6;
  if ((threadIdx.x & 63u) == 0) {
    wp[2 * w] = b1;
    wp[2 * w + 1] = b2;
  }
  __syncthreads();
  if (w != 0) return;
  const uint32_t l = threadIdx.x;
  b1 = l < 2 * nw ? wp[l] : 0;
  b2 = 0;
  top2_wave(b1, b2);
  if (l == 0 && b1) {
    unsigned long long* t = reinterpret_cast<unsigned long long*>(e->top);
    const uint64_t old = atomicMax(t, (unsigned long long)b1);
    if (old < b1) {
      if (old) atomicMax(t + 1, (unsigned long long)old);
      if (b2) atomicMax(t + 1, (unsigned long long)b2);
    } else {
      atomicMax(t + 1, (unsigned long long)b1);
    }
  }
}

__global__ __launch_bounds__(256, 1) void k_early(ShaArgs a, uint32_t split_bits) {
  extern __shared__ __attribute__((aligned(16))) uint32_t lds[];
  if (a.ctr->overflow || a.ctr->error) return;
  Early* e = a.early;
  const uint32_t wv = __builtin_amdgcn_readfirstlane(threadIdx.x >> 6);
  const uint32_t lane = threadIdx.x & 63u;
  for (uint32_t i = threadIdx.x; i < (uint32_t)kLongRow; i += blockDim.x) lds[kHelpOnes + i] = 1u;
  if (threadIdx.x < 8) lds[kHelpFlags + threadIdx.x] = 0u;
  __syncthreads();
  const uint32_t c = wv & 1u;
  ShaJob jb;
  uint32_t s;
  if (!early_key(a, (int)c, &s, &jb.start, &jb.end)) return;
  const uint64_t cn = a.cand[(uint32_t)e->top[c] + 1];
  const StreamDesc* sd = a.streams + s;
  jb.id = c;
  jb.stream = s;
  jb.level = cand_tz(cn) >= split_bits ? cand_tz(cn) - split_bits : 0u;
  jb.fin = 1;
  jb.prefix = 0;
  jb.consumed = 0;
  jb.dbase = a.data + sd->data_off + (jb.start - sd->seg_base);
  jb.hist = sd->hist + 64;
  jb.L = jb.end - jb.start;
  jb.nblocks = (uint32_t)((jb.L + 8) / 64 + 1);
  __builtin_amdgcn_s_setprio(3);
  if (wv >= 2) {
    solo_fill_blocks(a, jb, true, lds, c);
    return;
  }
  uint32_t st[8] = {0x6a09e667, 0xbb67ae85, 0x3c6ef372, 0xa54ff53a,
                    0x510e527f, 0x9b05688c, 0x1f83d9ab, 0x5be0cd19};
  const uint64_t tm0 = __builtin_amdgcn_s_memtime(), tr0 = __builtin_amdgcn_s_memrealtime();
  const uint32_t nb = __builtin_amdgcn_readfirstlane(jb.nblocks);
  if (!solo_chain_blocks(a, nb, st, lds, c)) return;
  if (lane == 0) {
    ChunkRec* r = e->rec + c;
    r->offset = jb.start;
    r->len = jb.L;
    r->level = jb.level;
    r->stream = jb.stream;
    uint32_t* ref = reinterpret_cast<uint32_t*>(r->ref);
#pragma unroll
    for (int i = 0; i < 8; ++i) ref[i] = __builtin_bswap32(st[i]);
    if (c == 0) {
      e->diag[1] = __builtin_amdgcn_s_memtime();
      e->diag[3] = __builtin_amdgcn_s_memrealtime();
      e->diag[0] = tm0;
      e->diag[2] = tr0;
      e->diag[4] = jb.nblocks;
    }
  }
}

__global__ void k_early_fix(Early* e, ChunkRec* out, Counters* ctr) {
  if (ctr->overflow || ctr->error) return;
  const int k = threadIdx.x;
  if (k < kEarly && e->top[k] && e->idx[k]) out[e->idx[k] - 1] = e->rec[k];
  if (k < kEarly && e->top[k] && !e->idx[k])
    atomicOr(reinterpret_cast<unsigned long long*>(&ctr->error), 16ull);
  if (k == 0 && e->top[0] && e->idx[0])
    for (int i = 0; i < 5; ++i) ctr->diag[i] = e->diag[i];
}

__global__ __launch_bounds__(256) void k_sha_blobs(BlobShaArgs a) {
  const uint64_t stride = (uint64_t)gridDim.x * blockDim.x;
  for (uint64_t i = (uint64_t)blockIdx.x * blockDim.x + threadIdx.x; i < a.n; i += stride) {
    ShaJob jb;
    jb.id = i;
    jb.start = 0;
    jb.end = a.len[i];
    jb.dbase = a.base + a.off[i];
    jb.hist = nullptr;
    jb.L = a.len[i];
    jb.consumed = 0;
    jb.prefix = 0;
    jb.fin = 1;
    jb.nblocks = (uint32_t)((jb.L + 8) / 64 + 1);
    uint32_t st[8] = {0x6a09e667, 0xbb67ae85, 0x3c6ef372, 0xa54ff53a,
                      0x510e527f, 0x9b05688c, 0x1f83d9ab, 0x5be0cd19};
    RawBlock rb;
    raw_load(jb.dbase, 0, 0, jb.L, rb);
    for (uint32_t blk = 0; blk < jb.nblocks; ++blk) {
      uint32_t W[16];
      raw_to_words(rb, W);
      if (rb.valid < 64) {
        pad_words(rb.valid, W);
        if (blk + 1 == jb.nblocks) {
// ... 208 lines not shown
```

bs_amd/csrc/bsgpu_launch.h:

```cpp
#pragma once
#include <hip/hip_runtime.h>
#include <stdint.h>

#include "bsgpu_internal.h"

namespace bsg {

struct ScanArgs {
  const uint8_t* data;
  const StreamDesc* streams;
  const uint64_t* strip0;
  uint32_t nstreams;
  uint64_t nstrips;
  const uint32_t* table;
  Params p;
  uint32_t* counts;
  uint64_t* refine;
  uint32_t* slots;
  const uint64_t* cand_off;
  uint64_t* cand;
  uint64_t cand_cap;
  Counters* ctr;
  uint32_t lists;
  uint64_t list_cap;
  uint32_t* list_cnt;
};
uint32_t scan_lists(uint64_t nstrips, int num_cus);
uint64_t scan_list_cap(uint64_t nstrips, uint32_t lists);

struct PrefixArgs {
  const uint32_t* in;
  uint64_t* out;
  uint64_t* partials;
  uint64_t n_bound;
  const uint64_t* n_dev;
  uint64_t* total;
  uint64_t* overflow;
  uint64_t cap;
  const uint64_t* skip_if;
  uint64_t* error;
};

struct SelArgs {
  const uint64_t* cand;
  const StreamDesc* streams;
  uint32_t* flags;
  Params p;
  Counters* ctr;
};

struct ChunkArgs {
  const uint64_t* cand;
  const uint32_t* flags;
  const uint64_t* fidx;
  uint64_t* bnd_end;
  uint64_t* bnd_info;
  uint64_t* scount;
  uint64_t* last_end;
  uint64_t chunk_cap;
  Params p;
  Counters* ctr;
  const StreamDesc* streams;
};

struct StartArgs {
  const StreamDesc* src;
  const uint64_t* src_strip0;
  StreamDesc* streams;
  uint64_t* strip0;
  uint32_t nstreams;
  uint64_t* last_end;
  uint64_t* scount;
  CarryOut* carry;
  uint32_t* zero0;
  uint32_t nzero0;
  uint32_t* zero1;
  uint32_t nzero1;
  uint32_t* zero2;
  uint32_t nzero2;
  uint32_t* zero3;
  uint32_t nzero3;
};

struct ShaArgs {
  const uint8_t* data;
  const StreamDesc* streams;
  uint32_t nstreams;
  const uint64_t* bnd_end;
  const uint64_t* bnd_info;
  const uint64_t* last_end;
  Counters* ctr;
  ChunkRec* out;
  CarryOut* carry;
  uint64_t chunk_cap;
  uint64_t* long_list;
  uint64_t* order;
  uint32_t* bucket_cnt;
  uint32_t* bucket_elig;
  uint32_t* bucket_off;
  uint32_t* bucket_loff;
  uint32_t* jinfo;
  LaneJob* jdesc;
  Regions* reg;
  uint8_t* oreg;
  uint64_t* rorder;
  uint64_t span;
  int long_mode;
  uint32_t waves;
  uint32_t seq_wait_limit;
  const uint64_t* cand;
  Early* early;
};

struct BlobShaArgs {
  const uint8_t* base;
  const uint64_t* off;
  const uint64_t* len;
  uint64_t n;
  uint8_t* refs;
};

hipError_t launch_scan(const ScanArgs& a, hipStream_t s, int num_cus);
hipError_t launch_compact(const ScanArgs& a, hipStream_t s, int num_cus);
hipError_t launch_rescan(const ScanArgs& a, hipStream_t s, int num_cus);
uint64_t prefix_partials_needed(uint64_t n_bound);
hipError_t launch_prefix(const PrefixArgs& a, hipStream_t s);
hipError_t launch_select(const SelArgs& a, uint64_t cand_bound, hipStream_t s, int num_cus);
hipError_t launch_chunks(const ChunkArgs& a, uint64_t cand_bound, uint32_t nstreams, hipStream_t s,
                         int num_cus);
hipError_t launch_start(const StartArgs& a, hipStream_t s);
hipError_t launch_blob_jobs(const ChunkArgs& a, const StreamDesc* streams, uint32_t nstreams,
                            hipStream_t s, int num_cus);
hipError_t launch_sha(const ShaArgs& a, uint64_t job_bound, hipStream_t s, int num_cus);
hipError_t launch_longlist(const ShaArgs& a, uint64_t job_bound, hipStream_t s, int num_cus);
hipError_t launch_lens(const ShaArgs& a, uint64_t job_bound, hipStream_t s, int num_cus);
hipError_t launch_order(const ShaArgs& a, uint64_t job_bound, hipStream_t s, int num_cus);

struct TailArgs {
  uint32_t* jinfo;
  const LaneJob* jdesc;
  Counters* ctr;
  uint64_t chunk_cap;
  TailHdr* hdr;
  TailItem* dlist;
  uint64_t* dsrc;
  uint64_t* hmeta;
  TailItem* hlist;
  uint32_t* hready;
  uint8_t* ring;
  uint64_t ring_bytes;
  uint32_t max_items;
  uint32_t force_cut;
  float us_per_block;
  float pcie_bytes_us;
  float host_bytes_us;
  float host1_bytes_us;
  const uint8_t* d_refs;
  ChunkRec* out;
};
hipError_t launch_tail_pick(const TailArgs& a, uint64_t job_bound, hipStream_t s, int num_cus);
hipError_t launch_tail_gather(const TailArgs& a, hipStream_t s);
hipError_t launch_tail_fix(const TailArgs& a, hipStream_t s);
hipError_t launch_sha_blobs(const BlobShaArgs& a, hipStream_t s, int num_cus);
hipError_t launch_pick(const uint64_t* cand, uint64_t cand_cap, Counters* ctr, uint32_t min_size,
                       Early* e, hipStream_t s, int num_cus);
hipError_t launch_early(const ShaArgs& a, uint32_t split_bits, hipStream_t s);
hipError_t launch_early_fix(Early* e, ChunkRec* out, Counters* ctr, hipStream_t s);
hipError_t launch_copy_out(const void* src, void* dst, uint64_t bytes, hipStream_t s);
hipError_t launch_fill_splitmix(uint8_t* p, uint64_t n, uint64_t seed, hipStream_t s,
                                int num_cus);

uint64_t sum_parts(uint64_t n);
hipError_t launch_ref_index(const PoolBlob* blobs, uint64_t nblobs, uint64_t* tab, uint64_t mask,
                            DedupHdr* hdr, hipStream_t s, int num_cus);

struct TreeArgs {
  const ChunkRec* rec;
  uint64_t M;
  const uint64_t* scount;
  uint32_t ns;
  uint32_t fanout;
  uint32_t H;
  uint32_t h;
  uint64_t nn;
  uint64_t arena_bytes;
  TreeHdr* hdr;
  uint64_t* cstart;
  uint32_t* rmax;
  uint8_t* kcnt;
  uint64_t* tmp;
  uint64_t* close;
  uint64_t* shbase;
  TreeNodeMeta* meta;
  uint64_t* pc;
  uint64_t* pn;
  uint64_t* aoff;
  uint64_t* part;
  uint8_t* arena;
  TreeNode* nodes;
  uint8_t* roots;
  uint64_t* ncount;
};
hipError_t launch_tree_count(const TreeArgs& a, hipStream_t s, int num_cus);
hipError_t launch_tree_layout(TreeArgs a, hipStream_t s, int num_cus);
hipError_t launch_tree_emit(const TreeArgs& a, uint64_t children, hipStream_t s, int num_cus);
hipError_t launch_tree_descs(const TreeArgs& a, uint64_t u0, uint32_t n, StreamDesc* d,
                             hipStream_t s, int num_cus);
hipError_t launch_tree_refs(const TreeArgs& a, uint64_t u0, uint32_t n, const ChunkRec* hashed,
                            const Counters* hctr, hipStream_t s, int num_cus);
hipError_t launch_tree_roots(const TreeArgs& a, hipStream_t s, int num_cus);

struct DedupArgs {
  const uint8_t* refs;
  uint64_t stride;
  const uint8_t* lens;
  uint64_t len_stride;
  uint64_t n;
  const uint8_t* refs2;
  const uint8_t* lens2;
  uint64_t n1;
  uint64_t* tab;
  uint64_t tab_mask;
  const uint8_t* set_keys;
  uint64_t set_stride;
  const uint64_t* set_tab;
  uint64_t set_mask;
  uint64_t set_count;
  uint64_t* first;
  uint64_t* rank;
  uint64_t* bpre;
  uint64_t* uniq;
  uint64_t* pack_off;
  uint64_t* part;
  DedupHdr* hdr;
};
hipError_t launch_dedup(const DedupArgs& a, hipStream_t s, int num_cus);

struct SetArgs {
  uint8_t* keys;
  uint64_t* tab;
  uint64_t mask;
  uint64_t count;
  DedupHdr* hdr;
};
hipError_t launch_set_rehash(const SetArgs& a, hipStream_t s, int num_cus);
hipError_t launch_set_add(const SetArgs& a, const DedupArgs& d, uint64_t m, hipStream_t s,
                          int num_cus);

struct PackArgs {
  const uint8_t* data;
  const StreamDesc* streams;
  uint32_t nstreams;
  const ChunkRec* rec;
  uint64_t nrec;
  const uint64_t* uniq;
  const uint64_t* pack_off;
  uint64_t nunique;
  uint64_t total;
  uint8_t* out;
  DedupHdr* hdr;
};
hipError_t launch_pack(const PackArgs& a, bool funnel, hipStream_t s);

struct RestoreArgs {
  const uint8_t* pool;
  uint64_t pool_bytes;
  const PoolBlob* blobs;
  uint64_t nblobs;
  const ChunkRec* rec;
  uint64_t nrec;
  const uint64_t* out_off;
  const uint64_t* out_len;
  const uint64_t* tpre;
  uint32_t ns;
  uint64_t* tab;
  uint64_t tab_mask;
  uint64_t* seg;
  uint64_t* sfirst;
  uint64_t* slast;
  uint8_t* out;
  RestoreHdr* hdr;
  const uint64_t* win0;
  uint8_t* touched;
};
hipError_t launch_restore_resolve(const RestoreArgs& a, bool index, hipStream_t s, int num_cus);
hipError_t launch_restore_descs(const RestoreArgs& a, uint64_t b0, uint32_t n, StreamDesc* d,
                                hipStream_t s, int num_cus);
hipError_t launch_restore_compare(const RestoreArgs& a, uint64_t b0, uint32_t n,
                                  const ChunkRec* hashed, const Counters* hctr, hipStream_t s,
                                  int num_cus);
hipError_t launch_restore_scatter(const RestoreArgs& a, uint64_t tiles, hipStream_t s);

struct WalkArgs {
  const uint8_t* pool;
  uint64_t pool_bytes;
  const PoolBlob* blobs;
  uint64_t nblobs;
  const uint8_t* roots;
  uint32_t ns;
  uint64_t* tab;
  uint64_t tab_mask;
  WalkHdr* hdr;
  uint64_t* sizes;
  uint32_t* status;
  uint32_t level;
  uint32_t last;
  uint64_t n;
  WalkItem* items;
  WalkNode* nodes;
// ... 171 lines not shown
```

bs_amd/csrc/bsgpu_tail.inc:

```

__device__ __forceinline__ bool tail_candidate(const TailArgs& a, uint64_t j, uint32_t floor,
                                               uint32_t* nb) {
  const uint32_t info = a.jinfo[j];
  if (info == kNoJob || !(info & kJobElig)) return false;
  *nb = info & ~kJobElig;
  if (*nb < floor) return false;
  return !(a.jdesc[j].meta & kLaneJobSlow);
}

__device__ __forceinline__ uint32_t tail_floor(const TailArgs& a) {
  return a.force_cut ? a.force_cut : kTailMinBlocks;
}

__device__ __forceinline__ uint32_t tail_bucket(uint64_t mx, uint32_t nb) {
  const uint64_t b = nb / (mx / kTailBuckets + 1);
  return b < kTailBuckets ? (uint32_t)b : kTailBuckets - 1;
}

__global__ __launch_bounds__(256) void k_offload_hist(TailArgs a) {
  __shared__ uint32_t cnt[kTailBuckets], mxb[kTailBuckets];
  __shared__ unsigned long long rb[kTailBuckets], nbk[kTailBuckets];
  if (a.ctr->overflow || a.ctr->error) return;
  const uint64_t M = a.ctr->nchunks;
  if (M > a.chunk_cap) return;
  const uint64_t mx = a.ctr->max_nblocks;
  const uint32_t floor = tail_floor(a);
  for (uint32_t i = threadIdx.x; i < kTailBuckets; i += blockDim.x) cnt[i] = mxb[i] = 0, rb[i] = nbk[i] = 0;
  __syncthreads();
  const uint64_t stride = (uint64_t)gridDim.x * blockDim.x;
  for (uint64_t j = (uint64_t)blockIdx.x * blockDim.x + threadIdx.x; j < M; j += stride) {
    uint32_t nb;
    if (!tail_candidate(a, j, floor, &nb)) continue;
    const uint32_t b = tail_bucket(mx, nb);
    atomicAdd(&cnt[b], 1u);
    atomicMax(&mxb[b], nb);
    atomicAdd(&rb[b], (unsigned long long)tail_slot(a.jdesc[j].len));
    atomicAdd(&nbk[b], (unsigned long long)nb);
  }
  __syncthreads();
  for (uint32_t b = threadIdx.x; b < kTailBuckets; b += blockDim.x)
    if (cnt[b]) {
      atomicAdd(&a.hdr->cnt[b], cnt[b]);
      atomicMax(&a.hdr->maxb[b], mxb[b]);
      atomicAdd(reinterpret_cast<unsigned long long*>(&a.hdr->rbytes[b]), rb[b]);
      atomicAdd(reinterpret_cast<unsigned long long*>(&a.hdr->nblk[b]), nbk[b]);
    }
}

__global__ void k_offload_cut(TailArgs a) {
  if (threadIdx.x != 0 || blockIdx.x != 0) return;
  TailHdr* h = a.hdr;
  const bool dead = a.ctr->overflow || a.ctr->error || a.ctr->nchunks > a.chunk_cap;
  const uint64_t mx = a.ctr->max_nblocks;
  uint64_t n = 0, B = 0, K = 0, low = kTailBuckets;
  uint64_t best_cut = kTailBuckets, best_n = 0, best_B = 0, best_K = 0, best_left = mx;
  float best_cost = (float)mx * a.us_per_block;
  const uint32_t floor = tail_floor(a);
  for (int b = (int)kTailBuckets - 1; b >= -1 && !dead; --b) {
    if (b >= 0 && h->cnt[b] == 0) continue;
    const uint64_t left = b >= 0 ? h->maxb[b] : min((uint64_t)(floor ? floor - 1 : 0), mx);
    if (n) {
      const float gpu = (float)left * a.us_per_block;
      const float rate = fminf(a.pcie_bytes_us, a.host_bytes_us);
      const float host = 30.f + (float)B / rate + (float)(mx * 64) / a.host1_bytes_us;
      const float cost = fmaxf(gpu, host);
      if (a.force_cut || cost < best_cost) {
        best_cost = cost;
        best_cut = low, best_n = n, best_B = B, best_K = K, best_left = left;
      }
    }
    if (b < 0) break;
    if (n + h->cnt[b] > a.max_items || B + h->rbytes[b] > a.ring_bytes) break;
    n += h->cnt[b], B += h->rbytes[b], K += h->nblk[b], low = (uint64_t)b;
  }
  uint32_t at = 0;
  for (int b = (int)kTailBuckets - 1; b >= (int)best_cut; --b) {
    h->base[b] = at;
    at += h->cnt[b];
  }
  h->count = best_n;
  h->cutb = best_cut;
  h->bytes = best_B;
  h->blocks = best_K;
  h->mx_all = mx;
  h->mx_left = best_left;
  if (best_n) {
    a.ctr->max_nblocks = best_left;
    a.ctr->total_blocks -= best_K;
  }
}

__global__ __launch_bounds__(256) void k_offload_take(TailArgs a) {
  TailHdr* h = a.hdr;
  if (h->count == 0) return;
  const uint64_t M = a.ctr->nchunks;
  const uint64_t mx = h->mx_all;
  const uint32_t floor = tail_floor(a), cutb = (uint32_t)h->cutb;
  const uint64_t stride = (uint64_t)gridDim.x * blockDim.x;
  for (uint64_t j = (uint64_t)blockIdx.x * blockDim.x + threadIdx.x; j < M; j += stride) {
    uint32_t nb;
    if (!tail_candidate(a, j, floor, &nb)) continue;
    const uint32_t b = tail_bucket(mx, nb);
    if (b < cutb) continue;
    const LaneJob d = a.jdesc[j];
    const uint64_t slot = tail_slot(d.len);
    const uint32_t i = h->base[b] + atomicAdd(&h->fill[b], 1u);
    const uint64_t off = atomicAdd(reinterpret_cast<unsigned long long*>(&h->ring_head),
                                   (unsigned long long)slot);
    if (i >= h->count || i >= a.max_items || off + slot > a.ring_bytes) {
      atomicOr(reinterpret_cast<unsigned long long*>(&a.ctr->error), 32ull);
      continue;
    }
    TailItem it;
    it.job = j;
    it.start = d.start;
    it.len = d.len;
    it.off = off + (d.dptr & 15u);
    it.stream = d.stream;
    it.level = d.meta & ~kLaneJobSlow;
    a.dlist[i] = it;
    a.dsrc[i] = d.dptr;
    a.jinfo[j] = kNoJob;
    atomicAdd(reinterpret_cast<unsigned long long*>(&h->taken), 1ull);
  }
}

__device__ __forceinline__ void store_release_system(uint32_t* p, uint32_t v) {
  __hip_atomic_store(p, v, __ATOMIC_RELEASE, __HIP_MEMORY_SCOPE_SYSTEM);
}

constexpr uint32_t kGatherThreads = 1024;
constexpr uint32_t kGatherWGs = 64;
__global__ __launch_bounds__(kGatherThreads) void k_offload_gather(TailArgs a) {
  const TailHdr* h = a.hdr;
  const bool ok = !a.ctr->overflow && !a.ctr->error && h->taken == h->count;
  const uint64_t n = ok ? min(h->count, (uint64_t)a.max_items) : 0;
  if (blockIdx.x == 0 && threadIdx.x == 0) {
    a.hmeta[1] = max(h->cutb * (h->mx_all / kTailBuckets + 1), (uint64_t)tail_floor(a));
    a.hmeta[2] = h->bytes;
    a.hmeta[3] = h->mx_all;
    a.hmeta[4] = h->mx_left;
    a.hmeta[5] = h->blocks;
    __hip_atomic_store(&a.hmeta[0], n, __ATOMIC_RELEASE, __HIP_MEMORY_SCOPE_SYSTEM);
  }
  for (uint64_t i = blockIdx.x; i < n; i += gridDim.x) {
    const TailItem it = a.dlist[i];
    if (it.off <= a.ring_bytes && it.len <= a.ring_bytes - it.off) {
      const uint8_t* src = reinterpret_cast<const uint8_t*>(a.dsrc[i]);
      uint8_t* dst = a.ring + it.off;
      const uint64_t head = min(it.len, (uint64_t)((16u - (uint32_t)(a.dsrc[i] & 15u)) & 15u));
      const uint64_t nvec = (it.len - head) / 16;
      const uint64_t tail0 = head + 16 * nvec;
      if (threadIdx.x < head) dst[threadIdx.x] = src[threadIdx.x];
      if (tail0 + threadIdx.x < it.len) dst[tail0 + threadIdx.x] = src[tail0 + threadIdx.x];
      const uint4* s4 = reinterpret_cast<const uint4*>(src + head);
      uint4* d4 = reinterpret_cast<uint4*>(dst + head);
      uint64_t v = threadIdx.x;
      for (; v + 3 * kGatherThreads < nvec; v += 4 * kGatherThreads) {
        const uint4 x0 = s4[v], x1 = s4[v + kGatherThreads], x2 = s4[v + 2 * kGatherThreads],
                    x3 = s4[v + 3 * kGatherThreads];
        d4[v] = x0;
        d4[v + kGatherThreads] = x1;
        d4[v + 2 * kGatherThreads] = x2;
        d4[v + 3 * kGatherThreads] = x3;
      }
      for (; v < nvec; v += kGatherThreads) d4[v] = s4[v];
    }
    if (threadIdx.x == 0) a.hlist[i] = it;
    __threadfence_system();
    __syncthreads();
    if (threadIdx.x == 0) store_release_system(a.hready + i, 1u);
  }
}

__global__ __launch_bounds__(256) void k_offload_fix(TailArgs a) {
  if (a.ctr->overflow || a.ctr->error) return;
  const uint64_t n = min(a.hdr->count, (uint64_t)a.max_items);
  for (uint64_t i = (uint64_t)blockIdx.x * blockDim.x + threadIdx.x; i < n;
       i += (uint64_t)gridDim.x * blockDim.x) {
    const TailItem it = a.dlist[i];
    if (it.job >= a.chunk_cap) continue;
    ChunkRec r;
    r.offset = it.start;
    r.len = it.len;
    r.level = it.level;
    r.stream = it.stream;
    for (int k = 0; k < 32; ++k) r.ref[k] = a.d_refs[32 * i + k];
    a.out[it.job] = r;
  }
}

hipError_t launch_tail_pick(const TailArgs& a, uint64_t job_bound, hipStream_t s, int num_cus) {
  const uint32_t grid = grid_for(job_bound, 256, 4u * (uint32_t)num_cus);
  hipLaunchKernelGGL(k_offload_hist, dim3(grid), dim3(256), 0, s, a);
  hipLaunchKernelGGL(k_offload_cut, dim3(1), dim3(64), 0, s, a);
  hipLaunchKernelGGL(k_offload_take, dim3(grid), dim3(256), 0, s, a);
  return hipGetLastError();
}

hipError_t launch_tail_gather(const TailArgs& a, hipStream_t s) {
  hipLaunchKernelGGL(k_offload_gather, dim3(kGatherWGs), dim3(kGatherThreads), 0, s, a);
  return hipGetLastError();
}

hipError_t launch_tail_fix(const TailArgs& a, hipStream_t s) {
  hipLaunchKernelGGL(k_offload_fix, dim3(16), dim3(256), 0, s, a);
  return hipGetLastError();
}
```

bs_amd/csrc/host_engine.h:

```cpp
#pragma once

namespace {

int normalize(const bsg_params* in, Params* out, bsg_params* norm) {
  bsg_params p = in ? *in : bsg_params_default();
  if (p.split_bits == 0) p.split_bits = 13;
  if (p.min_size == 0) p.min_size = 64;
  if (p.fanout == 0) p.fanout = 8;
  out->split_bits = p.split_bits;
  out->min_size = p.min_size;
  out->mask = p.split_bits >= 32 ? 0xffffffffu : ((1u << p.split_bits) - 1u);
  out->pad_ = 0;
  if (norm) *norm = p;
  return BSG_OK;
}

struct RunPlan {
  uint32_t ns = 0;
  uint64_t strips = 0;
  uint64_t total_len = 0;
  uint64_t data_span = 1;
  uint64_t cand_cap = 0;
  uint64_t chunk_cap = 0;
  uint32_t lists = 0;
  uint64_t list_cap = 0;
  uint64_t jobs = 0;
  bool scan = false;
  bool early = false;
  bool light = false;
  bool tail = false;
};

int device_error(uint64_t code) {
  std::fprintf(stderr, "bsgpu: device sanity check failed (code %llu)\n", (unsigned long long)code);
  return BSG_EDEVICE;
}

uint64_t data_span(const std::vector<StreamDesc>& descs) {
  uint64_t hi = 0;
  for (const StreamDesc& d : descs) hi = std::max<uint64_t>(hi, d.data_off + d.len);
  return hi;
}

struct RunView {
  bsg_engine* owner;
  hipStream_t stream;
  int num_cus, profile;
  bool run_done;
  bool usable;
  bool in_flight;
  const uint8_t* d_data;
  const std::vector<StreamDesc>* descs;
  StreamDesc* streams;
  uint32_t ns;
  ChunkRec* rec;
  uint64_t nrec, *scount;
  uint32_t fanout;
};

int need_hasher(bsg_engine* owner);
template <class Descs, class Consume>
int hash_batches(bsg_engine* owner, DevBuf& dbuf, uint64_t n, const uint8_t* data, uint64_t span,
                 int sha_mode, Descs descs, Consume consume);

}

#include "host_tree.h"
#include "host_dedup.h"
#include "host_restore.h"
#include "host_walk.h"
#include "host_gc.h"
#include "host_read.h"
#include "host_blobpool.h"
#include "host_blobs.h"

struct bsg_engine {
  int dev = 0;
  int num_cus = 256;
  hipStream_t stream = nullptr;
  DevBuf table, streams, strip0, counts, refine, slots, strip_off, partials_a, partials_b, cand, flags,
      fidx, bnd_end, bnd_info, scount, last_end, out, carry, ctr, long_list, order, buckets, jinfo, jdesc,
      regions, oreg, rorder;
  PinBuf h_streams, h_strip0, h_ctr;
  uint32_t htable[256];
  bool snapshot = false;
  PinBuf h_snap;
  Event sel_ev;
  const uint8_t* d_data = nullptr;
  std::vector<StreamDesc> descs;
  Params p{};
  uint64_t retry_cap = 0;
  uint32_t nstreams = 0;
  bool enqueued = false;
  bool hash_mode = false;
  int hash_long_mode = -1;
  Counters last{};
  int profile = 0;
  Marks marks;
  float stage_ms[3] = {0, 0, 0};
  hipStream_t estream = nullptr;
  Event cand_ev, pick_ev, early_ev;
  bool early_open = false;
  static constexpr uint64_t kEarlyMinBytes = 256ull << 20;
  uint64_t early_min = kEarlyMinBytes;
  bool early_ok() const {
    return !snapshot && !hash_mode && knob(BSG_KNOB_EARLY) != 0;
  }

  static constexpr uint64_t kTailMinBytes = 512ull << 20;
  static constexpr uint64_t kTailRingMax = 256ull << 20;
  static constexpr float kTailUsPerBlock = 0.95f;
  static constexpr float kTailPcieBytesUs = 56e3f;
  uint64_t tail_min = kTailMinBytes;
  uint32_t tail_force_cut = 0;
  bool tail_portable = false;
  uint64_t tail_ring_force = 0;
  std::unique_ptr<HashWorkers> workers;
  DevBuf tail_hdr, tail_list, tail_src, tail_refs;
  PinBuf h_tail, h_ring;
  Event tail_ev, gather_ev0, gather_ev1;
  bool tail_open = false;
  TailArgs tail_args{};
  int64_t tail_t0_ns = 0;
  struct TailStat {
    uint64_t chunks = 0, bytes = 0, cut = 0, longest_all = 0, longest_left = 0, blocks = 0;
    float gather_ms = 0.f;
    int64_t host_done_us = 0;
    int impl = 0, threads = 0;
    double host_rate = 0;
  } tail_stat;
  bool tail_ok() const {
    return !snapshot && !hash_mode && knob(BSG_KNOB_HOST_TAIL) != 0;
  }

  uint32_t fanout = 8;
  bool run_done = false;
  bool borrowed_stream = false;
  bsg_engine* hasher = nullptr;
  TreeWork tree;
  DedupWork dd;
  RestoreWork restore;
  WalkWork walk;
  GcWork gc;
  ReadWork read;
  MergeWork merge[2];
  BlobWork blobs;
  RunView view() {
    return RunView{this, stream, num_cus, profile, run_done, run_done && !snapshot && !hash_mode,
                   enqueued, d_data, &descs, streams.as<StreamDesc>(), nstreams,
                   out.as<ChunkRec>(), last.nchunks, scount.as<uint64_t>(), fanout};
  }


  void mark(int i, hipStream_t on = nullptr) {
    if (profile == 1 || (profile && i >= 2)) marks.record(i, on ? on : stream);
  }

  int setdev() { return herr(hipSetDevice(dev)); }

  RunPlan plan_split() {
    RunPlan pl;
    pl.scan = true;
    pl.ns = nstreams;
    pl.data_span = std::max<uint64_t>(1, data_span(descs));
    uint64_t chunk_bound = 0;
    for (uint32_t s = 0; s < pl.ns; ++s) {
      descs[s].strip0 = pl.strips;
      pl.strips += (descs[s].len + kStrip - 1) / kStrip;
      pl.total_len += descs[s].len;
      chunk_bound += (descs[s].len + (descs[s].seg_base - descs[s].open_start)) / p.min_size + 2;
    }
    {
      const uint32_t b = std::min<uint32_t>(p.split_bits, 16);
      pl.cand_cap = std::max<uint64_t>(1u << 16, ((pl.total_len >> b) << 2) + 2ull * pl.ns + 1024);
      if (retry_cap > pl.cand_cap) pl.cand_cap = retry_cap;
    }
    pl.chunk_cap = std::min(chunk_bound, pl.cand_cap);
    pl.lists = pl.strips ? scan_lists(pl.strips, num_cus) : 0;
    pl.list_cap = scan_list_cap(pl.strips, pl.lists);
    pl.jobs = pl.chunk_cap + pl.ns;
    pl.tail = tail_ok() && pl.total_len >= tail_min && pl.strips &&
              pl.total_len <= (uint64_t)knob(BSG_KNOB_LIGHT_BYTES).load();
    pl.early = !pl.tail && early_ok() && pl.total_len >= early_min && pl.strips;
    pl.light = pl.early && pl.total_len <= (uint64_t)knob(BSG_KNOB_LIGHT_BYTES).load();
    return pl;
  }

  RunPlan plan_hash() {
    RunPlan pl;
    pl.ns = nstreams;
    pl.data_span = std::max<uint64_t>(1, data_span(descs));
    pl.chunk_cap = pl.ns;
    pl.jobs = pl.chunk_cap + pl.ns;
    return pl;
  }

  static size_t ctr_bytes(const RunPlan& pl) {
    return sizeof(Counters) + (pl.scan ? sizeof(Early) : 0);
  }

  int reserve(const RunPlan& pl) {
    const uint64_t nn = pl.ns ? pl.ns : 1;
    const uint64_t recs = pl.scan ? pl.chunk_cap : nn;
    const uint64_t jobs = pl.scan ? pl.jobs : 2 * nn;
    if (pl.scan) {
      const uint64_t st = pl.strips ? pl.strips : 1;
      HCHECK(strip0.ensure(sizeof(uint64_t) * (pl.ns + 1)));
      HCHECK(counts.ensure(sizeof(uint32_t) * st));
      HCHECK(refine.ensure(sizeof(uint64_t) * (pl.lists * pl.list_cap + 1) +
                           sizeof(uint32_t) * (pl.lists + 1)));
      HCHECK(slots.ensure(sizeof(uint32_t) * kSlotCap * st));
      HCHECK(strip_off.ensure(sizeof(uint64_t) * st));
      HCHECK(partials_a.ensure(sizeof(uint64_t) * prefix_partials_needed(pl.strips)));
      HCHECK(partials_b.ensure(sizeof(uint64_t) * prefix_partials_needed(pl.cand_cap)));
      HCHECK(cand.ensure(sizeof(uint64_t) * pl.cand_cap));
      HCHECK(flags.ensure(sizeof(uint32_t) * pl.cand_cap));
      HCHECK(fidx.ensure(sizeof(uint64_t) * pl.cand_cap));
      HCHECK(h_strip0.ensure(sizeof(uint64_t) * (pl.ns + 1)));
    }
    HCHECK(streams.ensure(sizeof(StreamDesc) * nn));
    HCHECK(bnd_end.ensure(sizeof(uint64_t) * recs));
    HCHECK(bnd_info.ensure(sizeof(uint64_t) * recs));
    HCHECK(out.ensure(sizeof(ChunkRec) * recs));
    HCHECK(scount.ensure(sizeof(uint64_t) * nn));
    HCHECK(last_end.ensure(sizeof(uint64_t) * nn));
    HCHECK(carry.ensure(sizeof(CarryOut) * nn));
    HCHECK(ctr.ensure(ctr_bytes(pl)));
    HCHECK(long_list.ensure(sizeof(uint64_t) * jobs));
    HCHECK(order.ensure(sizeof(uint64_t) * jobs));
    HCHECK(jinfo.ensure(sizeof(uint32_t) * jobs));
    HCHECK(jdesc.ensure(sizeof(LaneJob) * jobs));
    HCHECK(regions.ensure(sizeof(Regions)));
    HCHECK(oreg.ensure(jobs));
    HCHECK(rorder.ensure(sizeof(uint64_t) * jobs));
    HCHECK(buckets.ensure(sizeof(uint32_t) * 4 * kLptBuckets));
    HCHECK(h_streams.ensure(sizeof(StreamDesc) * nn));
    HCHECK(h_ctr.ensure(sizeof(Counters)));
    return BSG_OK;
  }

  Counters* dctr() const { return ctr.as<Counters>(); }
  Early* dearly() const { return reinterpret_cast<Early*>(ctr.as<uint8_t>() + sizeof(Counters)); }

  StartArgs start_args(const RunPlan& pl) const {
    StartArgs a{};
    a.src = static_cast<const StreamDesc*>(h_streams.dev());
    a.streams = streams.as<StreamDesc>();
    a.nstreams = pl.ns;
    a.last_end = last_end.as<uint64_t>();
    a.scount = scount.as<uint64_t>();
    a.carry = carry.as<CarryOut>();
    a.zero0 = ctr.as<uint32_t>();
    a.nzero0 = (uint32_t)(ctr_bytes(pl) / 4);
    a.zero1 = buckets.as<uint32_t>();
    a.nzero1 = 2 * kLptBuckets;
    if (pl.scan) {
      a.src_strip0 = static_cast<const uint64_t*>(h_strip0.dev());
      a.strip0 = strip0.as<uint64_t>();
      a.zero2 = partials_a.as<uint32_t>();
      a.nzero2 = (uint32_t)(2 * prefix_partials_needed(pl.strips));
      a.zero3 = partials_b.as<uint32_t>();
      a.nzero3 = (uint32_t)(2 * prefix_partials_needed(pl.cand_cap));
    }
    return a;
  }

  ScanArgs scan_args(const RunPlan& pl) const {
    ScanArgs a{};
    a.data = d_data;
    a.streams = streams.as<StreamDesc>();
    a.strip0 = strip0.as<uint64_t>();
    a.nstreams = pl.ns;
    a.nstrips = pl.strips;
    a.table = table.as<uint32_t>();
    a.p = p;
    a.counts = counts.as<uint32_t>();
    a.refine = refine.as<uint64_t>();
    a.slots = slots.as<uint32_t>();
    a.cand_off = strip_off.as<uint64_t>();
    a.cand = cand.as<uint64_t>();
    a.cand_cap = pl.cand_cap;
    a.ctr = dctr();
// ... 48 lines not shown
    a.long_mode = long_mode;
    a.waves = 4u * (uint32_t)num_cus;
    a.seq_wait_limit = seq_wait_limit();
    a.cand = pl.scan ? cand.as<uint64_t>() : nullptr;
    a.early = early;
    return a;
  }

  int run_start(const RunPlan& pl, hipStream_t s) {
    std::memcpy(h_streams.p, descs.data(), sizeof(StreamDesc) * pl.ns);
    if (pl.scan) {
      uint64_t* h0 = h_strip0.as<uint64_t>();
      for (uint32_t k = 0; k < pl.ns; ++k) h0[k] = descs[k].strip0;
      h0[pl.ns] = pl.strips;
    }
    const StartArgs st = start_args(pl);
    if (!st.src || (pl.scan && !st.src_strip0)) return BSG_EDEVICE;
    HCHECK(dbg("launch_start", s, launch_start(st, s)));
    return BSG_OK;
  }

  int early_prepare() {
    if (!estream) HCHECK(stream_acquire(dev, &estream));
    const unsigned fl = hipEventDisableTiming | hipEventDisableSystemFence;
    HCHECK(cand_ev.create(fl));
    HCHECK(pick_ev.create(fl));
    HCHECK(early_ev.create(fl));
    return BSG_OK;
  }

  int run_scan(const RunPlan& pl, hipStream_t s) {
    const ScanArgs sa = scan_args(pl);
    mark(0);
    if (pl.strips) HCHECK(dbg("launch_scan", s, launch_scan(sa, s, num_cus)));
    mark(1);

    PrefixArgs pa{};
    pa.in = counts.as<uint32_t>();
    pa.out = strip_off.as<uint64_t>();
    pa.partials = partials_a.as<uint64_t>();
    pa.n_bound = pl.strips;
    pa.total = &dctr()->ncand;
    pa.overflow = &dctr()->overflow;
    pa.cap = pl.cand_cap;
    pa.error = &dctr()->error;
    HCHECK(dbg("launch_prefix", s, launch_prefix(pa, s)));

    if (pl.strips) HCHECK(dbg("launch_compact", s, launch_compact(sa, s, num_cus)));
    if (pl.strips) HCHECK(dbg("launch_rescan", s, launch_rescan(sa, s, num_cus)));
    return BSG_OK;
  }

  int run_pick(const RunPlan& pl, const ShaArgs& sh, hipStream_t s) {
    HCHECK(dbg("launch_pick", s,
               launch_pick(cand.as<uint64_t>(), pl.cand_cap, dctr(), p.min_size, dearly(), s,
                           num_cus)));
    HCHECK(hipEventRecord(pick_ev, s));
    HCHECK(dbg("launch_early", s, launch_early(sh, p.split_bits, s)));
    return BSG_OK;
  }

  int run_early(const RunPlan& pl, const ShaArgs& sh, hipStream_t* sel_stream) {
    int rc;
    if (pl.light) {
      if ((rc = run_pick(pl, sh, stream))) return rc;
      HCHECK(hipStreamWaitEvent(estream, pick_ev, 0));
      *sel_stream = estream;
      early_open = true;
    } else {
      HCHECK(hipEventRecord(cand_ev, stream));
      HCHECK(hipStreamWaitEvent(estream, cand_ev, 0));
      if ((rc = run_pick(pl, sh, estream))) return rc;
      HCHECK(hipEventRecord(early_ev, estream));
      early_open = true;
    }
    return BSG_OK;
  }

  int run_select(const RunPlan& pl, hipStream_t s) {
    SelArgs sel{cand.as<uint64_t>(), streams.as<StreamDesc>(), flags.as<uint32_t>(), p, dctr()};
    HCHECK(dbg("launch_select", s, launch_select(sel, pl.cand_cap, s, num_cus)));

    PrefixArgs pf{};
    pf.in = flags.as<uint32_t>();
    pf.out = fidx.as<uint64_t>();
    pf.partials = partials_b.as<uint64_t>();
    pf.n_bound = pl.cand_cap;
    pf.n_dev = &dctr()->ncand;
    pf.total = &dctr()->nchunks;
    pf.skip_if = &dctr()->overflow;
    pf.error = &dctr()->error;
    HCHECK(dbg("launch_prefix", s, launch_prefix(pf, s)));

    HCHECK(dbg("launch_chunks", s, launch_chunks(chunk_args(pl), pl.cand_cap, pl.ns, s, num_cus)));
    if (snapshot) {
      HCHECK(h_snap.ensure(sizeof(Counters) + 8ull * (pl.ns ? pl.ns : 1)));
      HCHECK(sel_ev.create(hipEventDisableTiming));
      uint8_t* hs = static_cast<uint8_t*>(h_snap.dev());
      if (!hs) return BSG_EDEVICE;
      HCHECK(launch_copy_out(ctr.p, hs, sizeof(Counters), stream));
      if (pl.ns) HCHECK(launch_copy_out(last_end.p, hs + sizeof(Counters), 8ull * pl.ns, stream));
      HCHECK(hipEventRecord(sel_ev, stream));
    }
    return BSG_OK;
  }

  static double host_sha_rate(bool portable) {
    static const double best = sha256_measure_rate(sha256_best_impl(), 256 << 10, 1.0);
    if (!portable || sha256_best_impl() == kShaPortable) return best;
    static const double plain = sha256_measure_rate(kShaPortable, 256 << 10, 1.0);
    return plain;
  }

  int tail_prepare(const RunPlan& pl) {
    if (!workers) workers.reset(new (std::nothrow) HashWorkers());
    if (!workers) return BSG_ENOMEM;
    if (!estream) HCHECK(stream_acquire(dev, &estream));
    HCHECK(tail_ev.create(hipEventDisableTiming | hipEventDisableSystemFence));
    HCHECK(gather_ev0.create());
    HCHECK(gather_ev1.create());
    const uint64_t ring =
        tail_ring_force ? tail_ring_force
                        : std::min<uint64_t>(kTailRingMax, std::max<uint64_t>(1 << 20, pl.total_len / 8));
    const uint32_t items = kTailMaxItems;
    HCHECK(h_ring.ensure(ring));
    const size_t meta = 64, flags = 4ull * items, list = sizeof(TailItem) * items;
    HCHECK(h_tail.ensure(meta + flags + list + 32ull * items));
    HCHECK(tail_hdr.ensure(sizeof(TailHdr)));
    HCHECK(tail_list.ensure(sizeof(TailItem) * items));
    HCHECK(tail_src.ensure(8ull * items));
    HCHECK(tail_refs.ensure(32ull * items));
    uint8_t* hd = static_cast<uint8_t*>(h_tail.dev());
    uint8_t* rd = static_cast<uint8_t*>(h_ring.dev());
    if (!hd || !rd) return BSG_EDEVICE;
    TailArgs& a = tail_args;
    a = TailArgs{};
    a.jinfo = jinfo.as<uint32_t>();
    a.jdesc = jdesc.as<LaneJob>();
    a.ctr = dctr();
    a.chunk_cap = pl.chunk_cap;
    a.hdr = tail_hdr.as<TailHdr>();
    a.dlist = tail_list.as<TailItem>();
    a.dsrc = tail_src.as<uint64_t>();
    a.hmeta = reinterpret_cast<uint64_t*>(hd);
    a.hready = reinterpret_cast<uint32_t*>(hd + meta);
    a.hlist = reinterpret_cast<TailItem*>(hd + meta + flags);
    a.ring = rd;
    a.ring_bytes = ring;
    a.max_items = items;
    a.force_cut = tail_force_cut;
    const double r1 = host_sha_rate(tail_portable);
    a.us_per_block = kTailUsPerBlock;
    a.pcie_bytes_us = kTailPcieBytesUs;
    a.host1_bytes_us = (float)(r1 * 1e-6);
    a.host_bytes_us = (float)(r1 * 1e-6 * workers->threads());
    a.d_refs = tail_refs.as<uint8_t>();
    a.out = out.as<ChunkRec>();
    tail_stat = TailStat{};
    tail_stat.host_rate = r1;
    tail_stat.threads = workers->threads();
    tail_stat.impl = tail_portable ? (int)kShaPortable : sha256_best_impl();
    return BSG_OK;
  }

  int run_tail_pick(const RunPlan& pl, hipStream_t s) {
    uint8_t* hp = h_tail.as<uint8_t>();
    uint64_t* meta = reinterpret_cast<uint64_t*>(hp);
    std::memset(hp, 0, 64 + 4ull * tail_args.max_items);
    meta[0] = kCountUnknown;
    HCHECK(hipMemsetAsync(tail_hdr.p, 0, sizeof(TailHdr), s));
    HCHECK(dbg("launch_tail_pick", s, launch_tail_pick(tail_args, pl.jobs, s, num_cus)));
    return BSG_OK;
  }

  int run_tail_gather(hipStream_t s) {
    uint8_t* hp = h_tail.as<uint8_t>();
    uint64_t* meta = reinterpret_cast<uint64_t*>(hp);
    HCHECK(hipEventRecord(tail_ev, s));
    HCHECK(hipStreamWaitEvent(estream, tail_ev, 0));
    HCHECK(hipEventRecord(gather_ev0, estream));
    HCHECK(dbg("launch_tail_gather", estream, launch_tail_gather(tail_args, estream)));
    HCHECK(hipEventRecord(gather_ev1, estream));
    static_assert(sizeof(HashItem) == sizeof(TailItem), "the list is the workers' items");
    HashBatch b;
    b.count = meta;
    b.ready = reinterpret_cast<const uint32_t*>(hp + 64);
    b.items = reinterpret_cast<const HashItem*>(hp + 64 + 4ull * tail_args.max_items);
    b.base = h_ring.as<uint8_t>();
    b.base_len = tail_args.ring_bytes;
    b.max_items = tail_args.max_items;
    b.refs = hp + 64 + (4ull + sizeof(TailItem)) * tail_args.max_items;
    b.impl = tail_stat.impl;
    tail_t0_ns = std::chrono::duration_cast<std::chrono::nanoseconds>(
                     std::chrono::steady_clock::now().time_since_epoch()).count();
    workers->start(b);
    tail_open = true;
    return BSG_OK;
  }

  int tail_settle() {
    if (!tail_open) return BSG_OK;
    tail_open = false;
    if (stream_wait(estream) != hipSuccess) {
      (void)hipGetLastError();
      workers->cancel();
      (void)workers->wait();
      return BSG_EDEVICE;
    }
    const uint64_t bad = workers->wait();
    const uint64_t* meta = h_tail.as<uint64_t>();
    const uint64_t n = std::min<uint64_t>(meta[0], tail_args.max_items);
    tail_stat.chunks = n;
    tail_stat.cut = n ? meta[1] : 0;
    tail_stat.bytes = n ? meta[2] : 0;
    tail_stat.longest_all = meta[3];
    tail_stat.longest_left = meta[4];
    tail_stat.blocks = n ? meta[5] : 0;
    if (hipEventElapsedTime(&tail_stat.gather_ms, gather_ev0, gather_ev1) != hipSuccess) {
      (void)hipGetLastError();
      tail_stat.gather_ms = -1.f;
    }
    tail_stat.host_done_us = n ? (workers->last_done_ns() - tail_t0_ns) / 1000 : 0;
    if (bad || workers->hashed_items() != n) return device_error(64);
    if (n) {
      const uint8_t* refs = h_tail.as<uint8_t>() + 64 + (4ull + sizeof(TailItem)) * tail_args.max_items;
      HCHECK(hipMemcpyAsync(tail_refs.p, refs, 32 * n, hipMemcpyHostToDevice, stream));
      HCHECK(dbg("launch_tail_fix", stream, launch_tail_fix(tail_args, stream)));
    }
    return BSG_OK;
  }

  int run_sha(const RunPlan& pl, const ShaArgs& sh, hipStream_t s) {
    if (pl.tail) {
      HCHECK(dbg("launch_lens", s, launch_lens(sh, pl.jobs, s, num_cus)));
      if (int rc = run_tail_pick(pl, s)) return rc;
      HCHECK(dbg("launch_order", s, launch_order(sh, pl.jobs, s, num_cus)));
      if (int rc = run_tail_gather(s)) return rc;
    } else
    HCHECK(dbg("launch_longlist", s, launch_longlist(sh, pl.jobs, s, num_cus)));
    mark(2, s);
    HCHECK(dbg("launch_sha", s, launch_sha(sh, pl.jobs, s, num_cus)));
    return BSG_OK;
  }

  int run_early_fix(const RunPlan& pl) {
    if (pl.light) HCHECK(hipEventRecord(early_ev, estream));
    HCHECK(hipStreamWaitEvent(stream, early_ev, 0));
    early_open = false;
    HCHECK(dbg("launch_early_fix", stream,
               launch_early_fix(dearly(), out.as<ChunkRec>(), dctr(), stream)));
    return BSG_OK;
  }

  int enqueue() {
    int rc;
    run_done = false;
    dd.valid = false;
    tree.valid = false;
    if (early_open) {
      HCHECK(hipStreamSynchronize(estream));
      early_open = false;
    }
    if ((rc = tail_settle())) return rc;
    const RunPlan pl = plan_split();
    if ((rc = reserve(pl)) || (rc = run_start(pl, stream))) return rc;
    if (pl.early && (rc = early_prepare())) return rc;
    if (pl.tail && (rc = tail_prepare(pl))) return rc;
    if (!pl.tail) tail_stat = TailStat{};
    const ShaArgs sh = sha_args(pl, long_mode(), pl.early ? dearly() : nullptr);
    if ((rc = run_scan(pl, stream))) return rc;
    hipStream_t sel_stream = stream;
    if (pl.early && (rc = run_early(pl, sh, &sel_stream))) return rc;
    if ((rc = run_select(pl, sel_stream))) return rc;
    if (pl.early && !pl.light) HCHECK(hipStreamWaitEvent(stream, pick_ev, 0));
    if ((rc = run_sha(pl, sh, sel_stream))) return rc;
    if (pl.early && (rc = run_early_fix(pl))) return rc;
    mark(3);
    enqueued = true;
    return BSG_OK;
  }

  int enqueue_hash() {
    int rc;
    run_done = false;
    dd.valid = false;
    tree.valid = false;
    if ((rc = tail_settle())) return rc;
    tail_stat = TailStat{};
    const RunPlan pl = plan_hash();
    if ((rc = reserve(pl)) || (rc = run_start(pl, stream))) return rc;
    mark(0);
    mark(1);
    if (pl.ns) HCHECK(dbg("launch_blob_jobs", stream,
                          launch_blob_jobs(chunk_args(pl), streams.as<StreamDesc>(), pl.ns, stream,
                                           num_cus)));
    const ShaArgs sh = sha_args(pl, hash_long_mode >= 0 ? hash_long_mode : long_mode(), nullptr);
    if ((rc = run_sha(pl, sh, stream))) return rc;
    mark(3);
    enqueued = true;
    return BSG_OK;
  }

  int finish(uint64_t* nchunks) {
    if (!enqueued) return BSG_ESTATE;
    for (int attempt = 0; attempt < 3; ++attempt) {
      if (int rc = tail_settle()) {
        enqueued = false;
        return rc;
      }
      HCHECK(hipMemcpyAsync(h_ctr.p, ctr.p, sizeof(Counters), hipMemcpyDeviceToHost, stream));
      HCHECK(stream_wait(stream));
      last = *h_ctr.as<Counters>();
      if (!last.overflow) break;
      retry_cap = last.ncand + 1024;
      int rc = hash_mode ? enqueue_hash() : enqueue();
      if (rc) return rc;
    }
    retry_cap = 0;
    if (last.overflow) return BSG_ENOMEM;
    enqueued = false;
    if (last.error) return device_error(last.error);
    if (profile)
      for (int i = 0; i < 3; ++i)
        stage_ms[i] = profile == 2 && i < 2 ? -1.f : marks.ms(i, i + 1, -1.f);
    if (nchunks) *nchunks = last.nchunks;
    run_done = !hash_mode && !snapshot;
    return BSG_OK;
  }

  int enqueue_hash_device(const uint8_t* data, uint64_t span, const StreamDesc* d_src,
                          uint32_t n, int sha_mode) {
    int rc;
    RunPlan pl;
    pl.ns = n;
    pl.data_span = std::max<uint64_t>(1, span);
    pl.chunk_cap = n;
    pl.jobs = 2ull * n;
    if ((rc = reserve(pl))) return rc;
    d_data = data;
    nstreams = n;
    hash_mode = true;
    normalize(nullptr, &p, nullptr);
    StartArgs st = start_args(pl);
    st.src = d_src;
    HCHECK(dbg("launch_start", stream, launch_start(st, stream)));
    HCHECK(dbg("launch_blob_jobs", stream,
               launch_blob_jobs(chunk_args(pl), streams.as<StreamDesc>(), pl.ns, stream, num_cus)));
    const ShaArgs sh = sha_args(pl, sha_mode, nullptr);
    return run_sha(pl, sh, stream);
  }
};

namespace {

int need_hasher(bsg_engine* owner) {
  if (owner->hasher) return BSG_OK;
  bsg_engine* h = new (std::nothrow) bsg_engine();
  if (!h) return BSG_ENOMEM;
  h->dev = owner->dev;
  h->num_cus = owner->num_cus;
  h->stream = owner->stream;
  h->borrowed_stream = true;
  owner->hasher = h;
  return BSG_OK;
}

template <class Descs, class Consume>
int hash_batches(bsg_engine* owner, DevBuf& dbuf, uint64_t n, const uint8_t* data, uint64_t span,
                 int sha_mode, Descs descs, Consume consume) {
  bsg_engine* hasher = owner->hasher;
  for (uint64_t b = 0; b < n; b += kTreeHashBatch) {
    const uint32_t nb = (uint32_t)std::min<uint64_t>(kTreeHashBatch, n - b);
    HCHECK(dbuf.ensure(sizeof(StreamDesc) * nb));
    HCHECK(descs(b, nb, dbuf.as<StreamDesc>()));
    if (int rc = hasher->enqueue_hash_device(data, span, dbuf.as<StreamDesc>(), nb, sha_mode))
// ... 8 lines not shown
```

bs_amd/csrc/host_sha256.cpp:

```cpp
#include "host_sha256.h"

#include <time.h>

#include <algorithm>
#include <chrono>
#include <cstdlib>
#include <cstring>

#if defined(__x86_64__) || defined(__i386__)
#define BSG_X86 1
#include <cpuid.h>
#include <immintrin.h>
#endif

namespace bsg {
namespace {

alignas(64) const uint32_t kK[64] = {
    0x428a2f98, 0x71374491, 0xb5c0fbcf, 0xe9b5dba5, 0x3956c25b, 0x59f111f1, 0x923f82a4, 0xab1c5ed5,
    0xd807aa98, 0x12835b01, 0x243185be, 0x550c7dc3, 0x72be5d74, 0x80deb1fe, 0x9bdc06a7, 0xc19bf174,
    0xe49b69c1, 0xefbe4786, 0x0fc19dc6, 0x240ca1cc, 0x2de92c6f, 0x4a7484aa, 0x5cb0a9dc, 0x76f988da,
    0x983e5152, 0xa831c66d, 0xb00327c8, 0xbf597fc7, 0xc6e00bf3, 0xd5a79147, 0x06ca6351, 0x14292967,
    0x27b70a85, 0x2e1b2138, 0x4d2c6dfc, 0x53380d13, 0x650a7354, 0x766a0abb, 0x81c2c92e, 0x92722c85,
    0xa2bfe8a1, 0xa81a664b, 0xc24b8b70, 0xc76c51a3, 0xd192e819, 0xd6990624, 0xf40e3585, 0x106aa070,
// ... 29 lines not shown
    }
    st[0] += a, st[1] += b, st[2] += c, st[3] += d, st[4] += e, st[5] += f, st[6] += g, st[7] += h;
  }
}

#ifdef BSG_X86
__attribute__((target("sha,sse4.1,ssse3")))
void blocks_x86(uint32_t st[8], const uint8_t* p, size_t nblocks) {
  const __m128i kSwap = _mm_set_epi64x(0x0c0d0e0f08090a0bll, 0x0405060700010203ll);
  __m128i t = _mm_shuffle_epi32(_mm_loadu_si128(reinterpret_cast<const __m128i*>(st)), 0xB1);
  __m128i s1 = _mm_shuffle_epi32(_mm_loadu_si128(reinterpret_cast<const __m128i*>(st + 4)), 0x1B);
  __m128i s0 = _mm_alignr_epi8(t, s1, 8);
  s1 = _mm_blend_epi16(s1, t, 0xF0);
  for (; nblocks; --nblocks, p += 64) {
    const __m128i save0 = s0, save1 = s1;
    __m128i m[4];
#pragma GCC unroll 16
    for (int g = 0; g < 16; ++g) {
      if (g < 4)
        m[g] = _mm_shuffle_epi8(_mm_loadu_si128(reinterpret_cast<const __m128i*>(p + 16 * g)), kSwap);
      __m128i kw = _mm_add_epi32(m[g & 3], _mm_load_si128(reinterpret_cast<const __m128i*>(kK + 4 * g)));
      s1 = _mm_sha256rnds2_epu32(s1, s0, kw);
      if (g >= 3 && g < 15) {
        const __m128i a = _mm_alignr_epi8(m[g & 3], m[(g + 3) & 3], 4);
        m[(g + 1) & 3] = _mm_sha256msg2_epu32(_mm_add_epi32(m[(g + 1) & 3], a), m[g & 3]);
      }
      kw = _mm_shuffle_epi32(kw, 0x0E);
      s0 = _mm_sha256rnds2_epu32(s0, s1, kw);
      if (g >= 1 && g < 13) m[(g + 3) & 3] = _mm_sha256msg1_epu32(m[(g + 3) & 3], m[g & 3]);
    }
    s0 = _mm_add_epi32(s0, save0);
    s1 = _mm_add_epi32(s1, save1);
  }
  t = _mm_shuffle_epi32(s0, 0x1B);
  s1 = _mm_shuffle_epi32(s1, 0xB1);
  s0 = _mm_blend_epi16(t, s1, 0xF0);
  s1 = _mm_alignr_epi8(s1, t, 8);
  _mm_storeu_si128(reinterpret_cast<__m128i*>(st), s0);
  _mm_storeu_si128(reinterpret_cast<__m128i*>(st + 4), s1);
}
#endif

void blocks(uint32_t st[8], const uint8_t* p, size_t nblocks, int impl) {
#ifdef BSG_X86
  if (impl == kShaX86) return blocks_x86(st, p, nblocks);
#endif
  (void)impl;
  blocks_portable(st, p, nblocks);
}

int64_t now_ns() {
  return std::chrono::duration_cast<std::chrono::nanoseconds>(
             std::chrono::steady_clock::now().time_since_epoch()).count();
}

inline void cpu_pause() {
#ifdef BSG_X86
  _mm_pause();
#endif
}

constexpr int64_t kSpinNs = 200'000;
template <class Pred>
bool poll_until(Pred pred, const std::atomic<bool>& stop) {
  const int64_t t0 = now_ns();
  bool spin = true;
  for (uint32_t it = 0;; ++it) {
    if (pred()) return true;
    if (stop.load(std::memory_order_acquire)) return false;
    if (spin && (it & 63u) == 63u && now_ns() - t0 >= kSpinNs) spin = false;
    if (spin) {
      for (int i = 0; i < 16; ++i) cpu_pause();
    } else {
      const timespec ts{0, 20'000};
      nanosleep(&ts, nullptr);
    }
  }
}

template <class T>
inline T load_acquire(const T* p) {
  return __atomic_load_n(p, __ATOMIC_ACQUIRE);
}

}

bool sha256_have_x86() {
#ifdef BSG_X86
  static const bool have = [] {
    unsigned a = 0, b = 0, c = 0, d = 0;
    if (!__get_cpuid(1, &a, &b, &c, &d)) return false;
    if (!(c & (1u << 9)) || !(c & (1u << 19))) return false;
    if (!__get_cpuid_count(7, 0, &a, &b, &c, &d)) return false;
    return (b & (1u << 29)) != 0;
  }();
  return have;
#else
  return false;
#endif
}

int sha256_best_impl() { return sha256_have_x86() ? kShaX86 : kShaPortable; }

const char* sha256_impl_name(int impl) { return impl == kShaX86 ? "x86-sha" : "portable"; }

void sha256_range(const uint8_t* p, size_t n, uint8_t out[32], int impl) {
  if (impl != kShaPortable) impl = sha256_best_impl();
  uint32_t st[8];
  std::memcpy(st, kInit, sizeof st);
  const size_t whole = n / 64;
  if (whole) blocks(st, p, whole, impl);
  uint8_t tail[128] = {0};
  const size_t rest = n - 64 * whole;
  if (rest) std::memcpy(tail, p + 64 * whole, rest);
  tail[rest] = 0x80;
  const size_t tb = rest + 9 <= 64 ? 1 : 2;
  const uint64_t bits = (uint64_t)n * 8;
  for (int i = 0; i < 8; ++i) tail[64 * tb - 1 - i] = (uint8_t)(bits >> (8 * i));
  blocks(st, tail, tb, impl);
  for (int i = 0; i < 8; ++i) {
    out[4 * i] = (uint8_t)(st[i] >> 24);
    out[4 * i + 1] = (uint8_t)(st[i] >> 16);
    out[4 * i + 2] = (uint8_t)(st[i] >> 8);
    out[4 * i + 3] = (uint8_t)st[i];
  }
}

double sha256_measure_rate(int impl, size_t bytes, double ms) {
  std::vector<uint8_t> buf(std::max<size_t>(bytes, 64));
  for (size_t i = 0; i < buf.size(); ++i) buf[i] = (uint8_t)(i * 2654435761u >> 24);
  uint8_t ref[32];
  sha256_range(buf.data(), buf.size(), ref, impl);
  const int64_t t0 = now_ns();
  uint64_t done = 0;
  int64_t t1 = t0;
  do {
    sha256_range(buf.data(), buf.size(), ref, impl);
    done += buf.size();
    t1 = now_ns();
  } while ((double)(t1 - t0) < ms * 1e6);
  return (double)done * 1e9 / (double)std::max<int64_t>(1, t1 - t0);
}

int HashWorkers::default_threads() {
  int n = 0;
  if (const char* e = std::getenv("OMP_NUM_THREADS")) n = std::atoi(e);
  if (n <= 0) n = (int)std::thread::hardware_concurrency();
  return std::max(1, std::min(16, n));
}

HashWorkers::HashWorkers(int threads) {
  const int n = threads > 0 ? std::min(16, threads) : default_threads();
  th_.reserve((size_t)n);
  for (int i = 0; i < n; ++i) th_.emplace_back([this] { loop(); });
}

HashWorkers::~HashWorkers() {
  if (open_) {
    cancel();
    (void)wait();
  }
  {
    std::lock_guard<std::mutex> g(mu_);
    quit_ = true;
  }
  cv_work_.notify_all();
  for (std::thread& t : th_) t.join();
}

void HashWorkers::start(const HashBatch& b) {
  std::lock_guard<std::mutex> g(mu_);
  cur_ = b;
  next_.store(0, std::memory_order_relaxed);
  bad_.store(0, std::memory_order_relaxed);
  nhashed_.store(0, std::memory_order_relaxed);
  last_ns_.store(0, std::memory_order_relaxed);
  cancel_.store(false, std::memory_order_relaxed);
  inside_ = (int)th_.size();
  open_ = true;
  ++gen_;
  cv_work_.notify_all();
}

void HashWorkers::cancel() { cancel_.store(true, std::memory_order_release); }

uint64_t HashWorkers::wait() {
  std::unique_lock<std::mutex> g(mu_);
  cv_done_.wait(g, [this] { return inside_ == 0; });
  open_ = false;
  return bad_.load(std::memory_order_relaxed);
}

void HashWorkers::loop() {
  uint64_t seen = 0;
  for (;;) {
    HashBatch b;
    {
      std::unique_lock<std::mutex> g(mu_);
      cv_work_.wait(g, [&] { return quit_ || gen_ != seen; });
      if (quit_) return;
      seen = gen_;
      b = cur_;
    }
    work(b);
    {
      std::lock_guard<std::mutex> g(mu_);
      if (--inside_ == 0) cv_done_.notify_all();
    }
  }
}

void HashWorkers::work(const HashBatch& b) {
  uint64_t n = kCountUnknown;
  if (!poll_until([&] { return (n = load_acquire(b.count)) != kCountUnknown; }, cancel_)) return;
  if (n > b.max_items) {
    bad_.fetch_add(1, std::memory_order_relaxed);
    n = b.max_items;
  }
  for (;;) {
    const uint64_t i = next_.fetch_add(1, std::memory_order_relaxed);
    if (i >= n) return;
    if (!poll_until([&] { return load_acquire(b.ready + i) != 0; }, cancel_)) return;
    const HashItem it = b.items[i];
    if (it.off > b.base_len || it.len > b.base_len - it.off) {
      bad_.fetch_add(1, std::memory_order_relaxed);
      continue;
    }
    sha256_range(b.base + it.off, (size_t)it.len, b.refs + 32 * i, b.impl);
    const int64_t t = now_ns();
    int64_t prev = last_ns_.load(std::memory_order_relaxed);
    while (prev < t && !last_ns_.compare_exchange_weak(prev, t, std::memory_order_relaxed)) {
    }
    nhashed_.fetch_add(1, std::memory_order_relaxed);
  }
}

}

extern "C" int bsg_host_sha256_debug(const uint8_t* p, uint64_t n, int impl, uint8_t out[32]) {
  if ((!p && n) || !out) return -1;
  if (impl == bsg::kShaX86 && !bsg::sha256_have_x86()) return 1;
  static const uint8_t none = 0;
  bsg::sha256_range(p ? p : &none, (size_t)n, out, impl);
  return 0;
}
```

bs_amd/csrc/host_sha256.h:

```cpp
#pragma once
#include <stddef.h>
#include <stdint.h>

#include <atomic>
#include <condition_variable>
#include <mutex>
#include <thread>
#include <vector>

namespace bsg {

enum ShaImpl : int { kShaAuto = -1, kShaPortable = 0, kShaX86 = 1 };

bool sha256_have_x86();
int sha256_best_impl();
const char* sha256_impl_name(int impl);
void sha256_range(const uint8_t* p, size_t n, uint8_t out[32], int impl = kShaAuto);
double sha256_measure_rate(int impl, size_t bytes, double ms);

struct HashItem {
  uint64_t job;
  uint64_t start;
  uint64_t len;
  uint64_t off;
  uint32_t stream;
  uint32_t level;
};
static_assert(sizeof(HashItem) == 40, "HashItem layout");

constexpr uint64_t kCountUnknown = ~0ull;
struct HashBatch {
  const uint64_t* count = nullptr;
  const HashItem* items = nullptr;
  const uint32_t* ready = nullptr;
  const uint8_t* base = nullptr;
  uint64_t base_len = 0;
  uint64_t max_items = 0;
  uint8_t* refs = nullptr;
  int impl = kShaAuto;
};

class HashWorkers {
 public:
  explicit HashWorkers(int threads = 0);
  ~HashWorkers();
  HashWorkers(const HashWorkers&) = delete;
  HashWorkers& operator=(const HashWorkers&) = delete;
  int threads() const { return (int)th_.size(); }
  static int default_threads();
  void start(const HashBatch& b);
  void cancel();
  uint64_t wait();
  bool busy() const { return open_; }
  int64_t last_done_ns() const { return last_ns_.load(std::memory_order_relaxed); }
  uint64_t hashed_items() const { return nhashed_.load(std::memory_order_relaxed); }

 private:
  void loop();
  void work(const HashBatch& b);
  std::vector<std::thread> th_;
  std::mutex mu_;
  std::condition_variable cv_work_, cv_done_;
  HashBatch cur_{};
  uint64_t gen_ = 0;
  int inside_ = 0;
  bool quit_ = false;
  bool open_ = false;
  std::atomic<bool> cancel_{false};
  std::atomic<uint64_t> next_{0}, bad_{0}, nhashed_{0};
  std::atomic<int64_t> last_ns_{0};
};

}
```

Before: 181.1.

## Price host-tail cut with tier-aware GPU model and calibrated host rate

Rewrites the tail offload-cut kernel as a wave-parallel scan over buckets. Each candidate cut is priced with a model that accounts for solo and group tier throughput and wave capacity, and the model also picks a larger solo-tier count that the ticket planner then uses. The host aggregate SHA rate is measured once with the worker pool, and the host start-up cost is raised to a more conservative estimate. Per-tier timestamps and per-worker host timing stats are added for diagnostics, which adds a few atomics and clock reads on hot paths.

Result: faster. 192.2, median of 6 (+6.1%).

```diff
diff --git a/bs_amd/bsgpu.py b/bs_amd/bsgpu.py
--- a/bs_amd/bsgpu.py
+++ b/bs_amd/bsgpu.py
@@ -351,6 +351,9 @@
         "bsg_engine_tiers_debug": (ctypes.c_int, [vp, u64p]),
         "bsg_engine_early_min_debug": (ctypes.c_int, [vp, ctypes.c_uint64]),
         "bsg_engine_host_tail": (ctypes.c_int, [vp, u64p]),
+        "bsg_engine_tail_plan_debug": (ctypes.c_int, [vp, ctypes.c_uint32, ctypes.c_int,
+                                                      ctypes.c_float, ctypes.c_float]),
+        "bsg_engine_tail_tiers_debug": (ctypes.c_int, [vp, u64p]),
         "bsg_engine_host_tail_debug": (ctypes.c_int, [vp, ctypes.c_uint64, ctypes.c_uint32,
                                                       ctypes.c_int, ctypes.c_uint64]),
         "bsg_host_sha256_debug": (ctypes.c_int, [vp, ctypes.c_uint64, ctypes.c_int, vp]),
@@ -1006,6 +1009,7 @@
                "nshort": int(d[13]), "wave_tickets": int(d[14]), "total_blocks": int(d[15])}
         t = np.zeros(4, dtype=np.uint64)
         _check(lib().bsg_engine_timeline(self.h, _p(t, ctypes.c_uint64)), "bsg_engine_timeline")
+        self._timeline0 = int(t[0])
         if t[0] and t[1] and t[3]:
             t0 = int(t[0])
             out["timeline_us"] = {"long_start": round((int(t[1]) - t0) * 0.01, 1),
@@ -1027,7 +1031,31 @@
                             "threads": int(t[6]), "host_rate_bytes_s": int(t[7]),
                             "longest_blocks": int(t[8]), "longest_left_blocks": int(t[9]),
                             "host_blocks": int(t[10]), "cpuid_sha": bool(t[11])}
+        p = np.zeros(67, dtype=np.uint64)
+        _check(lib().bsg_engine_tail_tiers_debug(self.h, _p(p, ctypes.c_uint64)),
+               "bsg_engine_tail_tiers_debug")
+        names = ("helped", "solo", "group", "pair", "lane")
+        out["solo_count"] = int(p[0])
+        out["num_cus"] = int(p[66])
+        out["tier_blocks"] = {k: int(p[6 + i]) for i, k in enumerate(names)}
+        if "timeline_us" in out:
+            t0 = int(self._timeline0)
+            out["timeline_us"]["tier_end"] = {k: round((int(p[1 + i]) - t0) * 0.01, 1)
+                                              for i, k in enumerate(names) if p[1 + i]}
+        nthr = out["host_tail"]["threads"]
+        out["host_tail"].update({
+            "solo_asked": int(p[11]), "plan_gpu_us": int(p[12]), "plan_host_us": int(p[13]),
+            "agg_rate_bytes_s": int(p[14]), "first_flag_us": int(p[15]),
+            "wait_us": int(p[16]), "hash_us": int(p[17]),
+            "workers": [{"wait_us": int(p[18 + 3 * i]), "hash_us": int(p[19 + 3 * i]),
+                         "bytes": int(p[20 + 3 * i])} for i in range(min(nthr, 16))]})
         return out
+
+    def set_tail_plan(self, solo: int = 0, legacy: bool = False, host_start_us: float = 0.0,
+                      host_bytes_us: float = 0.0) -> None:
+        _check(lib().bsg_engine_tail_plan_debug(self.h, int(solo), int(bool(legacy)),
+                                                float(host_start_us), float(host_bytes_us)),
+               "bsg_engine_tail_plan_debug")
 
     def set_host_tail(self, min_bytes: int = 512 << 20, force_cut: int = 0,
                       portable: bool = False, ring_bytes: int = 0) -> None:
diff --git a/bs_amd/csrc/bsgpu_host.cpp b/bs_amd/csrc/bsgpu_host.cpp
--- a/bs_amd/csrc/bsgpu_host.cpp
+++ b/bs_amd/csrc/bsgpu_host.cpp
@@ -1044,6 +1044,41 @@
   e->tail_force_cut = force_cut;
   e->tail_portable = portable != 0;
   e->tail_ring_force = ring_bytes;
+  return BSG_OK;
+}
+
+extern "C" int bsg_engine_tail_plan_debug(bsg_engine* e, uint32_t solo, int legacy,
+                                          float host_start_us, float host_bytes_us) {
+  if (!e || e->enqueued) return BSG_EINVAL;
+  e->tail_force_solo = solo;
+  e->tail_legacy = legacy != 0;
+  e->tail_host_start_force = host_start_us;
+  e->tail_host_rate_force = host_bytes_us;
+  return BSG_OK;
+}
+
+extern "C" int bsg_engine_tail_tiers_debug(const bsg_engine* e, uint64_t out[18 + 48 + 1]) {
+  if (!e || !out || e->enqueued) return BSG_EINVAL;
+  const bsg_engine::TailStat& t = e->tail_stat;
+  out[0] = e->last.solo;
+  for (uint32_t k = 0; k < kTiers; ++k) {
+    out[1 + k] = e->last.tier_end_rt[k];
+    out[6 + k] = e->last.tier_max[k];
+  }
+  if (e->last.tier_end_rt[kTierLane]) out[6 + kTierLane] = e->last.diag2[4];
+  out[11] = t.solo_asked;
+  out[12] = (uint64_t)std::max(0.f, t.plan_gpu_us);
+  out[13] = (uint64_t)std::max(0.f, t.plan_host_us);
+  out[14] = (uint64_t)t.agg_rate;
+  out[15] = (uint64_t)std::max<int64_t>(0, t.first_flag_us);
+  out[16] = (uint64_t)std::max<int64_t>(0, t.wait_us);
+  out[17] = (uint64_t)std::max<int64_t>(0, t.hash_us);
+  for (int i = 0; i < 16; ++i) {
+    out[18 + 3 * i] = (uint64_t)std::max<int64_t>(0, t.worker_us[i][0]);
+    out[19 + 3 * i] = (uint64_t)std::max<int64_t>(0, t.worker_us[i][1]);
+    out[20 + 3 * i] = t.worker_bytes[i];
+  }
+  out[66] = (uint64_t)e->num_cus;
   return BSG_OK;
 }
 
diff --git a/bs_amd/csrc/bsgpu_internal.h b/bs_amd/csrc/bsgpu_internal.h
--- a/bs_amd/csrc/bsgpu_internal.h
+++ b/bs_amd/csrc/bsgpu_internal.h
@@ -73,6 +73,8 @@
   uint32_t mask;
   uint32_t pad_;
 };
+
+enum Tier : uint32_t { kTierHelped = 0, kTierSolo, kTierGroup, kTierPair, kTierLane, kTiers };
 
 struct Counters {
   uint64_t ncand;
@@ -100,9 +102,12 @@
   uint64_t nrefine;
   uint64_t helped;
   uint64_t scan_ticket;
-  uint64_t pad[7];
-};
-static_assert(sizeof(Counters) == 320, "Counters layout");
+  uint64_t solo;
+  uint64_t tier_end_rt[kTiers];
+  uint64_t tier_max[kTiers];
+  uint64_t pad[4];
+};
+static_assert(sizeof(Counters) == 384, "Counters layout");
 
 struct LaneJob {
   uint64_t dptr;
@@ -160,6 +165,8 @@
   uint64_t mx_left;
   uint64_t ring_head;
   uint64_t taken;
+  float gpu_us, host_us;
+  uint64_t solo;
   uint32_t cnt[kTailBuckets];
   uint32_t maxb[kTailBuckets];
   uint64_t rbytes[kTailBuckets];
@@ -169,6 +176,9 @@
 };
 static_assert(sizeof(TailHdr) % 16 == 0, "TailHdr layout");
 constexpr uint32_t kTailMetaWords = 8;
+__host__ __device__ inline uint64_t tail_helper_extra(uint64_t helped) {
+  return 4 * ((helped + 1) / 2) - helped;
+}
 __host__ __device__ inline uint64_t tail_slot(uint64_t len) {
   return (len + 16 + kTailSlotAlign - 1) & ~(uint64_t)(kTailSlotAlign - 1);
 }
diff --git a/bs_amd/csrc/bsgpu_kernels.hip b/bs_amd/csrc/bsgpu_kernels.hip
--- a/bs_amd/csrc/bsgpu_kernels.hip
+++ b/bs_amd/csrc/bsgpu_kernels.hip
@@ -1436,13 +1436,29 @@
     }
     a.ctr->long_thresh = mx > (uint64_t)nlb * w ? mx - (uint64_t)nlb * w : 0;
     a.ctr->nlong_grp = n8;
-    a.ctr->tickets_grp = t8;
+    uint64_t S = kSolo, tS = t8;
+    const uint64_t npair_t = (nlong - n8 + kPairGroup - 1) / kPairGroup;
+    if (a.ctr->solo) {
+      const uint64_t hsolo = min(min((uint64_t)n8, (uint64_t)kSolo), (uint64_t)a.waves / 2);
+      const uint64_t other = npair_t + ((uint64_t)nshort + 63) / 64 + tail_helper_extra(hsolo);
+      uint64_t lo_s = min((uint64_t)kSolo, (uint64_t)n8);
+      uint64_t hi_s = min(max(a.ctr->solo, (uint64_t)kSolo), (uint64_t)n8);
+      while (lo_s < hi_s) {
+        const uint64_t mid = (lo_s + hi_s + 1) / 2;
+        if (mid + (n8 - mid + kGroup - 1) / kGroup + other <= a.waves) lo_s = mid;
+        else hi_s = mid - 1;
+      }
+      S = max(lo_s, (uint64_t)kSolo);
+      tS = n8 <= S ? n8 : S + (n8 - S + kGroup - 1) / kGroup;
+    }
+    a.ctr->solo = S;
+    a.ctr->tickets_grp = tS;
     const uint64_t helped = (light && a.long_mode == 0)
                                 ? min(min((uint64_t)n8, (uint64_t)kSolo), (uint64_t)a.waves / 2)
                                 : 0;
     a.ctr->helped = helped;
     a.ctr->long_head = helped;
-    a.ctr->ntickets = t8 + (nlong - n8 + kPairGroup - 1) / kPairGroup;
+    a.ctr->ntickets = tS + npair_t;
   }
 }
 
@@ -1535,13 +1551,21 @@
   return v;
 }
 
+__device__ __forceinline__ void tier_stamp(Counters* ctr, uint32_t tier, uint32_t nb) {
+  atomicMax(reinterpret_cast<unsigned long long*>(&ctr->tier_end_rt[tier]),
+            (unsigned long long)__builtin_amdgcn_s_memrealtime());
+  atomicMax(reinterpret_cast<unsigned long long*>(&ctr->tier_max[tier]), (unsigned long long)nb);
+}
+
+template <bool STAMP>
 __device__ void sha_wave_job(const ShaArgs& a, uint64_t M, uint64_t t, uint64_t nlong,
                              uint32_t* ring) {
   const uint32_t lane = threadIdx.x & 63u;
   const uint64_t n8 = a.ctr->nlong_grp, t8 = a.ctr->tickets_grp;
+  const uint64_t nsolo = a.ctr->solo;
   const bool pairs = t >= t8;
-  const bool solo = !pairs && t < kSolo;
-  const uint64_t j0 = solo ? t : pairs ? n8 + (t - t8) * kPairGroup : kSolo + (t - kSolo) * kGroup;
+  const bool solo = !pairs && t < nsolo;
+  const uint64_t j0 = solo ? t : pairs ? n8 + (t - t8) * kPairGroup : nsolo + (t - nsolo) * kGroup;
   const uint64_t jend = pairs ? nlong : n8;
   const uint32_t G = solo ? 1u : pairs ? kPairGroup : kGroup;
   const uint32_t B = 64u / G;
@@ -1637,6 +1661,8 @@
       a.ctr->diag[4] = jb.nblocks;
     }
   }
+  if constexpr (STAMP)
+    if (lane == 0) tier_stamp(a.ctr, solo ? kTierSolo : pairs ? kTierPair : kTierGroup, nmax);
 }
 
 __device__ __forceinline__ uint64_t pop_uniform(uint64_t* head) {
@@ -1726,6 +1752,7 @@
       a.ctr->diag[2] = tr0;
       a.ctr->diag[4] = jb.nblocks;
     }
+    tier_stamp(a.ctr, kTierHelped, nb);
   }
 }
 
@@ -1834,18 +1861,22 @@
     for (uint32_t i = threadIdx.x & 63u; i < (uint32_t)kLongRow; i += 64) ring[64 * kLongRow + i] = 1u;
     t = pop_uniform(&a.ctr->long_head);
   }
+  const bool ticketed = helper_wg || t < ntickets;
   if (t < ntickets) {
     __builtin_amdgcn_s_setprio(3);
     while (t < ntickets) {
-      sha_wave_job(a, M, t, nlong, ring);
+      sha_wave_job<HELP>(a, M, t, nlong, ring);
       t = pop_uniform(&a.ctr->long_head);
     }
     __builtin_amdgcn_s_setprio(0);
   }
   sha_lane_mode(a, M);
-  if ((threadIdx.x & 63u) == 0)
+  if ((threadIdx.x & 63u) == 0) {
     atomicMax(reinterpret_cast<unsigned long long*>(&a.ctr->lane_end_rt),
               (unsigned long long)__builtin_amdgcn_s_memrealtime());
+    if constexpr (HELP)
+      if (!ticketed) tier_stamp(a.ctr, kTierLane, 0);
+  }
 }
 
 __device__ __forceinline__ uint64_t pick_key(const uint64_t* __restrict__ cand, uint64_t n,
diff --git a/bs_amd/csrc/bsgpu_launch.h b/bs_amd/csrc/bsgpu_launch.h
--- a/bs_amd/csrc/bsgpu_launch.h
+++ b/bs_amd/csrc/bsgpu_launch.h
@@ -155,6 +155,11 @@
   float pcie_bytes_us;
   float host_bytes_us;
   float host1_bytes_us;
+  float us_solo, us_group;
+  float host_start_us;
+  uint32_t waves;
+  uint32_t force_solo;
+  uint32_t legacy_model;
   const uint8_t* d_refs;
   ChunkRec* out;
 };
diff --git a/bs_amd/csrc/bsgpu_tail.inc b/bs_amd/csrc/bsgpu_tail.inc
--- a/bs_amd/csrc/bsgpu_tail.inc
+++ b/bs_amd/csrc/bsgpu_tail.inc
@@ -47,46 +47,157 @@
     }
 }
 
-__global__ void k_offload_cut(TailArgs a) {
-  if (threadIdx.x != 0 || blockIdx.x != 0) return;
+struct CutPrice {
+  float gpu, host;
+  uint32_t solo;
+};
+
+__device__ __forceinline__ CutPrice cut_price(const TailArgs& a, const uint32_t* sn, uint64_t mx,
+                                              uint64_t M, uint64_t left, uint32_t n, uint64_t B) {
+  CutPrice p;
+  const float rate = fminf(a.pcie_bytes_us, a.host_bytes_us);
+  p.host = a.host_start_us + (float)B / rate + (float)(mx * 64) / a.host1_bytes_us;
+  p.solo = kSolo;
+  if (a.legacy_model) {
+    p.gpu = (float)left * a.us_per_block;
+    return p;
+  }
+  const uint32_t floor = tail_floor(a);
+  const uint32_t rem = sn[0] - n;
+  auto at_least = [&](uint64_t x) { return x < floor ? rem : sn[tail_bucket(mx, (uint32_t)x)] - n; };
+  const float D = (float)left * (rem > kSolo ? fmaxf(a.us_solo, a.us_per_block) : a.us_per_block);
+  p.gpu = D;
+  const uint64_t tl = max(left * BSG_TLEN_PCT_LIGHT / 100, (uint64_t)kLongMinBlocks);
+  const uint64_t tl2 = max(left * BSG_PAIR_PCT_LIGHT / 100, (uint64_t)kLongMinBlocks);
+  const uint64_t thr = (uint64_t)(D / a.us_group);
+  const uint32_t want = max(thr >= left ? 0u : at_least(thr + 1), kSolo);
+  const uint64_t n8 = at_least(tl), nl = max((uint64_t)at_least(tl2), n8);
+  const uint64_t lanes = M > n + nl ? (M - n - nl + 63) / 64 : 0;
+  const uint64_t other = (nl - n8 + kPairGroup - 1) / kPairGroup + lanes + tail_helper_extra(min(n8, (uint64_t)kSolo));
+  const uint64_t R = a.waves > other ? a.waves - other : 0;
+  const uint64_t fit = n8 <= R ? n8 : 8 * R > n8 + 7 ? (8 * R - n8 - 7) / 7 : 0;
+  if (want <= fit || want <= kSolo) {
+    p.solo = want;
+    return p;
+  }
+  p.solo = (uint32_t)max(fit, (uint64_t)kSolo);
+  uint32_t lo = 0, hi = kTailBuckets;
+  if (rem > p.solo) {
+    while (hi - lo > 1) {
+      const uint32_t mid = (lo + hi) / 2;
+      if (sn[mid] > n + p.solo) lo = mid;
+      else hi = mid;
+    }
+    const uint64_t top = min(left, (uint64_t)(lo + 1) * (mx / kTailBuckets + 1) - 1);
+    p.gpu = fmaxf(p.gpu, (float)top * a.us_group);
+  } else {
+    p.gpu = fmaxf(p.gpu, (float)min((uint64_t)floor, left) * a.us_group);
+  }
+  return p;
+}
+
+__global__ __launch_bounds__(64) void k_offload_cut(TailArgs a) {
+  __shared__ uint32_t sn[kTailBuckets + 1];
+  if (blockIdx.x != 0) return;
+  const uint32_t lane = threadIdx.x;
   TailHdr* h = a.hdr;
   const bool dead = a.ctr->overflow || a.ctr->error || a.ctr->nchunks > a.chunk_cap;
-  const uint64_t mx = a.ctr->max_nblocks;
-  uint64_t n = 0, B = 0, K = 0, low = kTailBuckets;
-  uint64_t best_cut = kTailBuckets, best_n = 0, best_B = 0, best_K = 0, best_left = mx;
+  const uint64_t mx = a.ctr->max_nblocks, M = a.ctr->nchunks;
+  const uint32_t floor = tail_floor(a);
+  uint32_t c[4], m[4];
+  uint64_t rb[4], nk[4];
+#pragma unroll
+  for (int i = 0; i < 4; ++i) {
+    c[i] = h->cnt[4 * lane + i];
+    m[i] = h->maxb[4 * lane + i];
+    rb[i] = h->rbytes[4 * lane + i];
+    nk[i] = h->nblk[4 * lane + i];
+  }
+  uint32_t own_low = kTailBuckets;
+#pragma unroll
+  for (int i = 3; i >= 0; --i)
+    if (c[i]) own_low = 4 * lane + i;
+  uint32_t xn = c[0] + c[1] + c[2] + c[3], xlow = own_low;
+  uint64_t xB = rb[0] + rb[1] + rb[2] + rb[3], xK = nk[0] + nk[1] + nk[2] + nk[3];
+  const uint32_t on = xn;
+  const uint64_t oB = xB, oK = xK;
+  for (uint32_t o = 1; o < 64; o <<= 1) {
+    const uint32_t tn = (uint32_t)__shfl_down((int)xn, o), tl = (uint32_t)__shfl_down((int)xlow, o);
+    const uint64_t tB = (uint64_t)__shfl_down((long long)xB, o);
+    const uint64_t tK = (uint64_t)__shfl_down((long long)xK, o);
+    if (lane + o < 64) xn += tn, xB += tB, xK += tK, xlow = min(xlow, tl);
+  }
+  uint32_t upn = xn - on;
+  uint64_t upB = xB - oB, upK = xK - oK;
+  uint32_t uplow = (uint32_t)__shfl_down((int)xlow, 1);
+  if (lane == 63) uplow = kTailBuckets;
+  uint32_t an[4], alow[4];
+  uint64_t aB[4], aK[4];
+#pragma unroll
+  for (int i = 3; i >= 0; --i) {
+    an[i] = upn, aB[i] = upB, aK[i] = upK, alow[i] = uplow;
+    sn[4 * lane + i] = upn + c[i];
+    upn += c[i], upB += rb[i], upK += nk[i];
+    if (c[i]) uplow = 4 * lane + i;
+  }
+  if (lane == 0) sn[kTailBuckets] = 0;
+  __syncthreads();
   float best_cost = (float)mx * a.us_per_block;
-  const uint32_t floor = tail_floor(a);
-  for (int b = (int)kTailBuckets - 1; b >= -1 && !dead; --b) {
-    if (b >= 0 && h->cnt[b] == 0) continue;
-    const uint64_t left = b >= 0 ? h->maxb[b] : min((uint64_t)(floor ? floor - 1 : 0), mx);
-    if (n) {
-      const float gpu = (float)left * a.us_per_block;
-      const float rate = fminf(a.pcie_bytes_us, a.host_bytes_us);
-      const float host = 30.f + (float)B / rate + (float)(mx * 64) / a.host1_bytes_us;
-      const float cost = fmaxf(gpu, host);
-      if (a.force_cut || cost < best_cost) {
-        best_cost = cost;
-        best_cut = low, best_n = n, best_B = B, best_K = K, best_left = left;
-      }
-    }
-    if (b < 0) break;
-    if (n + h->cnt[b] > a.max_items || B + h->rbytes[b] > a.ring_bytes) break;
-    n += h->cnt[b], B += h->rbytes[b], K += h->nblk[b], low = (uint64_t)b;
-  }
-  uint32_t at = 0;
-  for (int b = (int)kTailBuckets - 1; b >= (int)best_cut; --b) {
-    h->base[b] = at;
-    at += h->cnt[b];
-  }
-  h->count = best_n;
-  h->cutb = best_cut;
-  h->bytes = best_B;
-  h->blocks = best_K;
-  h->mx_all = mx;
-  h->mx_left = best_left;
-  if (best_n) {
-    a.ctr->max_nblocks = best_left;
-    a.ctr->total_blocks -= best_K;
+  float b_gpu = 0.f, b_host = 0.f;
+  uint32_t b_solo = 0, b_n = 0, b_cut = kTailBuckets;
+  int b_at = 256;
+  uint64_t b_B = 0, b_K = 0, b_left = mx;
+  auto consider = [&](int b, uint32_t n, uint64_t B, uint64_t K, uint32_t low, uint64_t left) {
+    if (dead || n == 0 || n > a.max_items || B > a.ring_bytes) return;
+    const CutPrice p = cut_price(a, sn, mx, M, left, n, B);
+    const float cost = fmaxf(p.gpu, p.host);
+    if (a.force_cut || cost < best_cost) {
+      best_cost = cost;
+      b_at = b, b_n = n, b_B = B, b_K = K, b_cut = low, b_left = left;
+      b_gpu = p.gpu, b_host = p.host, b_solo = p.solo;
+    }
+  };
+#pragma unroll
+  for (int i = 3; i >= 0; --i)
+    if (c[i]) consider((int)(4 * lane + i), an[i], aB[i], aK[i], alow[i], m[i]);
+  if (lane == 0) consider(-1, upn, upB, upK, uplow, min((uint64_t)(floor ? floor - 1 : 0), mx));
+  float w_cost = best_cost;
+  int w_at = b_at;
+  for (int o = 32; o > 0; o >>= 1) {
+    const float oc = __shfl_xor(w_cost, o);
+    const int oa = __shfl_xor(w_at, o);
+    const bool take = a.force_cut ? oa < w_at
+                                  : (oa != 256 && (w_at == 256 || oc < w_cost || (oc == w_cost && oa > w_at)));
+    if (take) w_cost = oc, w_at = oa;
+  }
+  const bool mine = w_at != 256 && w_at == b_at;
+  const uint32_t best_cut = (uint32_t)__shfl((int)b_cut, w_at == 256 ? 0 : (w_at < 0 ? 0 : w_at / 4));
+  const uint32_t cutb = w_at == 256 ? kTailBuckets : best_cut;
+#pragma unroll
+  for (int i = 0; i < 4; ++i)
+    if (4 * lane + i >= cutb) h->base[4 * lane + i] = an[i];
+  if (w_at == 256 && lane == 0) {
+    h->count = 0;
+    h->cutb = kTailBuckets;
+    h->bytes = 0;
+    h->blocks = 0;
+    h->mx_all = mx;
+    h->mx_left = mx;
+  }
+  if (mine) {
+    h->count = b_n;
+    h->cutb = b_cut;
+    h->bytes = b_B;
+    h->blocks = b_K;
+    h->mx_all = mx;
+    h->mx_left = b_left;
+    h->gpu_us = b_gpu;
+    h->host_us = b_host;
+    const uint32_t solo = a.force_solo ? a.force_solo : b_solo;
+    h->solo = solo;
+    a.ctr->max_nblocks = b_left;
+    a.ctr->total_blocks -= b_K;
+    a.ctr->solo = solo;
   }
 }
 
@@ -141,6 +252,8 @@
     a.hmeta[3] = h->mx_all;
     a.hmeta[4] = h->mx_left;
     a.hmeta[5] = h->blocks;
+    a.hmeta[6] = ((uint64_t)__float_as_uint(h->host_us) << 32) | __float_as_uint(h->gpu_us);
+    a.hmeta[7] = h->solo;
     __hip_atomic_store(&a.hmeta[0], n, __ATOMIC_RELEASE, __HIP_MEMORY_SCOPE_SYSTEM);
   }
   for (uint64_t i = blockIdx.x; i < n; i += gridDim.x) {
diff --git a/bs_amd/csrc/host_engine.h b/bs_amd/csrc/host_engine.h
--- a/bs_amd/csrc/host_engine.h
+++ b/bs_amd/csrc/host_engine.h
@@ -111,10 +111,21 @@
   static constexpr uint64_t kTailRingMax = 256ull << 20;
   static constexpr float kTailUsPerBlock = 0.95f;
   static constexpr float kTailPcieBytesUs = 56e3f;
+  static constexpr float kTailUsSolo = 1.075f;
+  static constexpr float kTailUsGroup = 1.39f;
+  static constexpr float kTailHostStartUs = 350.f;
+  static constexpr uint64_t kTailCalibBytes = 2ull << 20;
   uint64_t tail_min = kTailMinBytes;
   uint32_t tail_force_cut = 0;
   bool tail_portable = false;
   uint64_t tail_ring_force = 0;
+  uint32_t tail_force_solo = 0;
+  bool tail_legacy = false;
+  float tail_host_start_force = 0;
+  float tail_host_rate_force = 0;
+  double tail_agg_rate = 0;
+  int tail_agg_impl = -1;
+  int tail_stat_impl() const { return tail_portable ? (int)kShaPortable : sha256_best_impl(); }
   std::unique_ptr<HashWorkers> workers;
   DevBuf tail_hdr, tail_list, tail_src, tail_refs;
   PinBuf h_tail, h_ring;
@@ -128,6 +139,13 @@
     int64_t host_done_us = 0;
     int impl = 0, threads = 0;
     double host_rate = 0;
+    double agg_rate = 0;
+    float plan_gpu_us = 0, plan_host_us = 0;
+    uint64_t solo_asked = 0;
+    int64_t first_flag_us = 0;
+    int64_t wait_us = 0, hash_us = 0;
+    int64_t worker_us[16][2] = {};
+    uint64_t worker_bytes[16] = {};
   } tail_stat;
   bool tail_ok() const {
     return !snapshot && !hash_mode && knob(BSG_KNOB_HOST_TAIL) != 0;
@@ -482,12 +500,28 @@
     const double r1 = host_sha_rate(tail_portable);
     a.us_per_block = kTailUsPerBlock;
     a.pcie_bytes_us = kTailPcieBytesUs;
+    if (tail_agg_rate <= 0 || tail_agg_impl != tail_stat_impl()) {
+      tail_agg_impl = tail_stat_impl();
+      const uint64_t calib = std::min<uint64_t>(ring, kTailCalibBytes * (uint64_t)workers->threads());
+      std::memset(h_ring.as<uint8_t>(), 0x5a, calib);
+      tail_agg_rate = workers->measure_rate(h_ring.as<uint8_t>(), calib, tail_stat_impl());
+      if (tail_agg_rate <= 0) tail_agg_rate = r1 * workers->threads();
+    }
     a.host1_bytes_us = (float)(r1 * 1e-6);
-    a.host_bytes_us = (float)(r1 * 1e-6 * workers->threads());
+    a.host_bytes_us = (float)((tail_legacy ? r1 * workers->threads() : tail_agg_rate) * 1e-6);
+    a.us_solo = kTailUsSolo;
+    a.us_group = kTailUsGroup;
+    a.host_start_us = tail_legacy ? 30.f : kTailHostStartUs;
+    if (tail_host_start_force > 0) a.host_start_us = tail_host_start_force;
+    if (tail_host_rate_force > 0) a.pcie_bytes_us = a.host_bytes_us = tail_host_rate_force;
+    a.waves = sha_args(pl, 0, nullptr).waves;
+    a.force_solo = tail_force_solo;
+    a.legacy_model = tail_legacy ? 1u : 0u;
     a.d_refs = tail_refs.as<uint8_t>();
     a.out = out.as<ChunkRec>();
     tail_stat = TailStat{};
     tail_stat.host_rate = r1;
+    tail_stat.agg_rate = tail_agg_rate;
     tail_stat.threads = workers->threads();
     tail_stat.impl = tail_portable ? (int)kShaPortable : sha256_best_impl();
     return BSG_OK;
@@ -551,6 +585,24 @@
       tail_stat.gather_ms = -1.f;
     }
     tail_stat.host_done_us = n ? (workers->last_done_ns() - tail_t0_ns) / 1000 : 0;
+    if (n) {
+      uint32_t gb, hb;
+      gb = (uint32_t)meta[6], hb = (uint32_t)(meta[6] >> 32);
+      std::memcpy(&tail_stat.plan_gpu_us, &gb, 4);
+      std::memcpy(&tail_stat.plan_host_us, &hb, 4);
+      tail_stat.solo_asked = meta[7];
+      int64_t first = 0;
+      for (int i = 0; i < workers->threads(); ++i) {
+        const HashWorkers::WorkerStat& w = workers->stat(i);
+        tail_stat.worker_us[i][0] = w.wait_ns / 1000;
+        tail_stat.worker_us[i][1] = w.hash_ns / 1000;
+        tail_stat.worker_bytes[i] = w.bytes;
+        tail_stat.wait_us += w.wait_ns / 1000;
+        tail_stat.hash_us += w.hash_ns / 1000;
+        if (w.first_ns && (!first || w.first_ns < first)) first = w.first_ns;
+      }
+      tail_stat.first_flag_us = first ? (first - tail_t0_ns) / 1000 : 0;
+    }
     if (bad || workers->hashed_items() != n) return device_error(64);
     if (n) {
       const uint8_t* refs = h_tail.as<uint8_t>() + 64 + (4ull + sizeof(TailItem)) * tail_args.max_items;
diff --git a/bs_amd/csrc/host_sha256.cpp b/bs_amd/csrc/host_sha256.cpp
--- a/bs_amd/csrc/host_sha256.cpp
+++ b/bs_amd/csrc/host_sha256.cpp
@@ -205,7 +205,7 @@
 HashWorkers::HashWorkers(int threads) {
   const int n = threads > 0 ? std::min(16, threads) : default_threads();
   th_.reserve((size_t)n);
-  for (int i = 0; i < n; ++i) th_.emplace_back([this] { loop(); });
+  for (int i = 0; i < n; ++i) th_.emplace_back([this, i] { loop(i); });
 }
 
 HashWorkers::~HashWorkers() {
@@ -229,10 +229,48 @@
   nhashed_.store(0, std::memory_order_relaxed);
   last_ns_.store(0, std::memory_order_relaxed);
   cancel_.store(false, std::memory_order_relaxed);
+  for (WorkerStat& w : stat_) w = WorkerStat{};
   inside_ = (int)th_.size();
   open_ = true;
   ++gen_;
   cv_work_.notify_all();
+}
+
+double HashWorkers::measure_rate(const uint8_t* base, uint64_t bytes, int impl) {
+  const uint64_t n = (uint64_t)th_.size();
+  const uint64_t piece = (bytes / n) & ~(uint64_t)63;
+  {
+    std::lock_guard<std::mutex> g(mu_);
+    if (open_) return 0;
+  }
+  if (!base || !piece) return 0;
+  std::vector<HashItem> items(n);
+  std::vector<uint32_t> ready(n, 1u);
+  std::vector<uint8_t> refs(32 * n);
+  for (uint64_t i = 0; i < n; ++i) items[i] = HashItem{i, 0, piece, i * piece, 0, 0};
+  const uint64_t count = n;
+  HashBatch b;
+  b.count = &count;
+  b.items = items.data();
+  b.ready = ready.data();
+  b.base = base;
+  b.base_len = n * piece;
+  b.max_items = n;
+  b.refs = refs.data();
+  b.impl = impl;
+  double best = 0;
+  for (int round = 0; round < 5; ++round) {
+    start(b);
+    if (wait() || hashed_items() != n) return 0;
+    int64_t t0 = 0, t1 = 0;
+    for (const WorkerStat& w : stat_) {
+      if (!w.items) continue;
+      if (!t0 || w.first_ns < t0) t0 = w.first_ns;
+      if (w.last_ns > t1) t1 = w.last_ns;
+    }
+    if (round && t1 > t0) best = std::max(best, (double)(n * piece) * 1e9 / (double)(t1 - t0));
+  }
+  return best;
 }
 
 void HashWorkers::cancel() { cancel_.store(true, std::memory_order_release); }
@@ -244,7 +282,7 @@
   return bad_.load(std::memory_order_relaxed);
 }
 
-void HashWorkers::loop() {
+void HashWorkers::loop(int id) {
   uint64_t seen = 0;
   for (;;) {
     HashBatch b;
@@ -255,7 +293,7 @@
       seen = gen_;
       b = cur_;
     }
-    work(b);
+    work(b, stat_[id]);
     {
       std::lock_guard<std::mutex> g(mu_);
       if (--inside_ == 0) cv_done_.notify_all();
@@ -263,7 +301,7 @@
   }
 }
 
-void HashWorkers::work(const HashBatch& b) {
+void HashWorkers::work(const HashBatch& b, WorkerStat& ws) {
   uint64_t n = kCountUnknown;
   if (!poll_until([&] { return (n = load_acquire(b.count)) != kCountUnknown; }, cancel_)) return;
   if (n > b.max_items) {
@@ -273,7 +311,11 @@
   for (;;) {
     const uint64_t i = next_.fetch_add(1, std::memory_order_relaxed);
     if (i >= n) return;
+    const int64_t tw = now_ns();
     if (!poll_until([&] { return load_acquire(b.ready + i) != 0; }, cancel_)) return;
+    const int64_t th = now_ns();
+    ws.wait_ns += th - tw;
+    if (!ws.first_ns) ws.first_ns = th;
     const HashItem it = b.items[i];
     if (it.off > b.base_len || it.len > b.base_len - it.off) {
       bad_.fetch_add(1, std::memory_order_relaxed);
@@ -281,6 +323,10 @@
     }
     sha256_range(b.base + it.off, (size_t)it.len, b.refs + 32 * i, b.impl);
     const int64_t t = now_ns();
+    ws.hash_ns += t - th;
+    ws.bytes += it.len;
+    ws.items += 1;
+    ws.last_ns = t;
     int64_t prev = last_ns_.load(std::memory_order_relaxed);
     while (prev < t && !last_ns_.compare_exchange_weak(prev, t, std::memory_order_relaxed)) {
     }
diff --git a/bs_amd/csrc/host_sha256.h b/bs_amd/csrc/host_sha256.h
--- a/bs_amd/csrc/host_sha256.h
+++ b/bs_amd/csrc/host_sha256.h
@@ -54,10 +54,17 @@
   bool busy() const { return open_; }
   int64_t last_done_ns() const { return last_ns_.load(std::memory_order_relaxed); }
   uint64_t hashed_items() const { return nhashed_.load(std::memory_order_relaxed); }
+  struct WorkerStat {
+    int64_t wait_ns = 0, hash_ns = 0, first_ns = 0, last_ns = 0;
+    uint64_t bytes = 0, items = 0;
+  };
+  const WorkerStat& stat(int i) const { return stat_[i]; }
+  double measure_rate(const uint8_t* base, uint64_t bytes, int impl);
 
  private:
-  void loop();
-  void work(const HashBatch& b);
+  void loop(int id);
+  void work(const HashBatch& b, WorkerStat& ws);
+  WorkerStat stat_[16];
   std::vector<std::thread> th_;
   std::mutex mu_;
   std::condition_variable cv_work_, cv_done_;
```
